# CompVis/stable-diffusion

Hardware: AMD Instinct MI355X
Metric: 512x512 images/sec, SD-v1-4 50-step PLMS CFG=7.5 (higher is better)
Workload: dtype f16

## Files before the change

### include/sdmi.h

```cpp
#ifndef SDMI_H_
#define SDMI_H_

#include <stdint.h>

#ifdef __cplusplus
extern "C" {
#endif

#define SDMI_ABI_VERSION 17

typedef struct sdmi_unet sdmi_unet;

typedef struct sdmi_unet_cfg {
  int32_t in_channels;
  int32_t out_channels;
  int32_t model_channels;
  int32_t num_res_blocks;
  int32_t n_levels;
  int32_t channel_mult[8];
  int32_t n_attention_resolutions;
  int32_t attention_resolutions[8];
  int32_t num_heads;
  int32_t transformer_depth;
  int32_t context_dim;
} sdmi_unet_cfg;

const char* sdmi_last_error(void);
int sdmi_abi_version(void);
int sdmi_has_experiments(void);

int sdmi_unet_create(const sdmi_unet_cfg* cfg, sdmi_unet** out);
#define SDMI_PRECISION_MIXED 0
#define SDMI_PRECISION_FULL 1
int sdmi_unet_create_with_precision(const sdmi_unet_cfg* cfg, int precision, sdmi_unet** out);
int sdmi_unet_precision(const sdmi_unet* h);
typedef struct sdmi_unet_ext {
  int32_t attention_block;
  int32_t resblock_updown;
} sdmi_unet_ext;
int sdmi_unet_create_ext(const sdmi_unet_cfg* cfg, const sdmi_unet_ext* ext, int precision, sdmi_unet** out);
#define SDMI_UNET_SCALE_SHIFT_NORM 1u
#define SDMI_UNET_NUM_HEAD_CHANNELS_SHIFT 16
#define SDMI_UNET_NUM_HEAD_CHANNELS_MASK 0x0fff0000u
#define SDMI_UNET_NUM_HEAD_CHANNELS(n) (((unsigned)(n) << SDMI_UNET_NUM_HEAD_CHANNELS_SHIFT) & SDMI_UNET_NUM_HEAD_CHANNELS_MASK)
int sdmi_unet_create_flags(const sdmi_unet_cfg* cfg, const sdmi_unet_ext* ext, unsigned flags, int precision, sdmi_unet** out);
int sdmi_unet_destroy(sdmi_unet* h);
int sdmi_unet_num_weights(const sdmi_unet* h);
int sdmi_unet_weight_info(const sdmi_unet* h, int idx, char* key_buf, int key_buf_len, int64_t* shape4, int* ndim);
int sdmi_unet_set_weight(sdmi_unet* h, const char* key, const float* ptr, const int64_t* shape, int ndim, void* stream);
int sdmi_unet_finalize(sdmi_unet* h);

int64_t sdmi_unet_packed_bytes(sdmi_unet* h);
int sdmi_unet_export_packed(sdmi_unet* h, void* host_buf, int64_t bytes, void* stream);
int sdmi_unet_import_packed(sdmi_unet* h, const void* host_buf, int64_t bytes, void* stream);

int64_t sdmi_unet_workspace_bytes(sdmi_unet* h, int B, int H, int W, int Lctx);

int sdmi_unet_cache_context(sdmi_unet* h, const float* ctx, int B, int Lctx, void* workspace, int64_t workspace_bytes,
                            void* stream);
int sdmi_unet_reserve_context(sdmi_unet* h, int B, int Lctx);

int sdmi_unet_cache_timesteps(sdmi_unet* h, const int64_t* t_host, int n, void* stream);
int sdmi_unet_hint_timestep(sdmi_unet* h, int64_t t);
int sdmi_unet_tape_stats(sdmi_unet* h, int64_t* replayed, int64_t* recorded);

int sdmi_unet_forward(sdmi_unet* h, const float* x, const int64_t* t_i64, const float* t_f32, const float* ctx,
                      float* eps_out, int B, int H, int W, int Lctx, void* workspace, int64_t workspace_bytes,
                      void* stream);

int sdmi_sampler_step(const float* eps_model, int cfg, float scale, const float* x, int mode, const float* old0,
                      const float* old1, const float* old2, float a_t, float a_prev, float sigma, float sqrt_1m_at,
                      const float* noise, float* e_t_out, float* x_prev, float* pred_x0, int64_t n, void* stream);


int sdmi_dpm_solver_step(const float* eps_model, int cfg, float scale, const float* x, const float* m_prev, float alpha_s,
                         float sigma_s, float cx, float a, float inv_r0, int order, float* m_out, float* x_next, int64_t n,
                         void* stream);

typedef struct sdmi_vae sdmi_vae;
typedef struct sdmi_vae_cfg {
  int32_t ch;
  int32_t out_ch;
  int32_t n_levels;
  int32_t ch_mult[8];
  int32_t num_res_blocks;
  int32_t in_channels;
  int32_t z_channels;
  int32_t embed_dim;
} sdmi_vae_cfg;
int sdmi_vae_create(const sdmi_vae_cfg* cfg, int parts, sdmi_vae** out);
typedef struct sdmi_vae_ext {
  int32_t double_z;
  int32_t mid_attn;
  int32_t n_embed;
} sdmi_vae_ext;
int sdmi_vae_create_ext(const sdmi_vae_cfg* cfg, const sdmi_vae_ext* ext, int parts, sdmi_vae** out);
int sdmi_vae_create_precision(const sdmi_vae_cfg* cfg, const sdmi_vae_ext* ext, int parts, int precision, sdmi_vae** out);
int sdmi_vae_precision(const sdmi_vae* h);
int sdmi_vae_decode_vq(sdmi_vae* h, const float* z, float z_scale, int quantize, float* img, int B, int H, int W, void* workspace,
                       int64_t workspace_bytes, void* stream);
int sdmi_vae_destroy(sdmi_vae* h);
int sdmi_vae_num_weights(const sdmi_vae* h);
int sdmi_vae_weight_info(const sdmi_vae* h, int idx, char* key_buf, int key_buf_len, int64_t* shape4, int* ndim);
int sdmi_vae_set_weight(sdmi_vae* h, const char* key, const float* ptr, const int64_t* shape, int ndim, void* stream);
int sdmi_vae_finalize(sdmi_vae* h);
int64_t sdmi_vae_decode_workspace_bytes(sdmi_vae* h, int B, int H, int W);
int sdmi_vae_decode(sdmi_vae* h, const float* z, float z_scale, float* img, int B, int H, int W, void* workspace,
                    int64_t workspace_bytes, void* stream);
int64_t sdmi_vae_encode_workspace_bytes(sdmi_vae* h, int B, int H, int W);
int sdmi_vae_encode(sdmi_vae* h, const float* img, float* moments, int B, int H, int W, void* workspace,
                    int64_t workspace_bytes, void* stream);


typedef struct sdmi_clip sdmi_clip;
typedef struct sdmi_clip_cfg {
  int32_t vocab_size;
  int32_t hidden_size;
  int32_t intermediate_size;
  int32_t num_layers;
  int32_t num_heads;
  int32_t max_positions;
} sdmi_clip_cfg;
int sdmi_clip_create(const sdmi_clip_cfg* cfg, sdmi_clip** out);
int sdmi_clip_destroy(sdmi_clip* h);
int sdmi_clip_num_weights(const sdmi_clip* h);
int sdmi_clip_weight_info(const sdmi_clip* h, int idx, char* key_buf, int key_buf_len, int64_t* shape4, int* ndim);
int sdmi_clip_set_weight(sdmi_clip* h, const char* key, const float* ptr, const int64_t* shape, int ndim, void* stream);
int sdmi_clip_finalize(sdmi_clip* h);
int64_t sdmi_clip_workspace_bytes(sdmi_clip* h, int B, int L);
int sdmi_clip_forward(sdmi_clip* h, const int64_t* ids, float* out, int B, int L, void* workspace, int64_t workspace_bytes,
                      void* stream);

typedef struct sdmi_bert sdmi_bert;
typedef struct sdmi_bert_cfg {
  int32_t vocab_size;
  int32_t dim;
  int32_t depth;
  int32_t heads;
  int32_t dim_head;
  int32_t ff_inner;
  int32_t max_seq_len;
} sdmi_bert_cfg;
int sdmi_bert_create(const sdmi_bert_cfg* cfg, sdmi_bert** out);
int sdmi_bert_destroy(sdmi_bert* h);
int sdmi_bert_num_weights(const sdmi_bert* h);
int sdmi_bert_weight_info(const sdmi_bert* h, int idx, char* key_buf, int key_buf_len, int64_t* shape4, int* ndim);
int sdmi_bert_set_weight(sdmi_bert* h, const char* key, const float* ptr, const int64_t* shape, int ndim, void* stream);
int sdmi_bert_finalize(sdmi_bert* h);
int64_t sdmi_bert_workspace_bytes(sdmi_bert* h, int B, int L);
int sdmi_bert_forward(sdmi_bert* h, const int64_t* ids, float* out, int B, int L, void* workspace, int64_t workspace_bytes,
                      void* stream);

typedef struct sdmi_igemm_desc {
  const void* a0; const void* a1; const void* a2;
  int32_t c0, c1, c2, lda0, lda1, lda2;
  int32_t B, Hin, Win, Hout, Wout, ksize, stride, up;
  const void* w;
  int32_t N;
  int32_t mode;
  const float* bias; const float* rowvec; int32_t ld_rowvec;
  const float* residual; int32_t ldr;
  float* out_f32; void* out_f16; int32_t ldo;
  void* seg_dst[3]; int32_t seg_kind[3];
  int32_t heads, dh, ntok, ntok_pad, segC;
  int32_t splitk;
  float* splitk_ws; int64_t splitk_ws_floats;
  int32_t tile;
  int32_t dma;
  int32_t asym_pad;
  int32_t gn_n; void* gn_acc[2]; int32_t gn_cpg[2]; int32_t gn_cbase[2];
  int32_t* splitk_cnt; int32_t splitk_cnt_ints;
  int32_t split16;
  const float* f16_scale; float* lnp_out;
  const float* lnf_part; int32_t lnf_npart; float lnf_eps; const float* lnf_cs; const float* lnf_d;
  const float* pgn_gamma; const float* pgn_beta; float pgn_eps; int32_t pgn_silu;
  void* pgn_out; int32_t pgn_keep_f32; int32_t* pgn_applied;
  void* out_lo;
} sdmi_igemm_desc;
int sdmi_k_igemm(const sdmi_igemm_desc* d, void* stream);
int sdmi_k_ff_tail(const sdmi_igemm_desc* proj_out, const void* ln_f16, const float* lnp, float ln_eps, const float* csd,
                   const void* wgg_f16, const void* wff2_f16, const float* bff2, const float* t, void* stream);
int sdmi_k_st_tail(const sdmi_igemm_desc* proj_out, const void* a_f16, const void* wo_f16, const float* bo, float* t, const float* ln_gamma,
                   float ln_eps, const float* csd, const void* wgg_f16, const void* wff2_f16, const float* bff2, void* stream);
int sdmi_k_gn_conv3(const sdmi_igemm_desc* conv, const float* x0, const float* x1, int c0, int c1, float* gn_ws, int64_t gn_ws_floats,
                    const float* gn_gamma, const float* gn_beta, float gn_eps, void* stream);
int sdmi_k_st_head(const float* x, float* gn_ws, int64_t gn_ws_floats, const float* gn_gamma, const float* gn_beta, float gn_eps,
                   const void* w_in3, const float* b_in, float* t, const float* ln_gamma, float ln_eps, const void* wqkv_f16,
                   const float* lnf_cs, const float* lnf_d, void* q, void* k, void* vt, int B, int ntok, int ntok_pad, int heads, int dh,
                   int C, void* stream);
int sdmi_k_st_mid(const void* a_f16, const void* wo_f16, const float* bo, float* t, const float* ln_gamma, float ln_eps, const void* wq_f16,
                  const float* lnf_cs, const float* lnf_d, void* q, int B, int ntok, int heads, int dh, int C, void* stream);
int sdmi_k_st_mid_ctx(const void* a_f16, const void* wo_f16, const float* bo, float* t, const float* ln_gamma, float ln_eps, const void* wq_f16,
                      const float* lnf_cs, const float* lnf_d, const void* ctx_k, const void* ctx_vt, int nkv, int nkv_pad, float scale, void* ao_out,
                      int B, int ntok, int heads, int dh, int C, void* stream);
int sdmi_k_ln_fold_prep(const void* w_f16, int N, int K, int ldw, const float* gamma, const float* beta, const float* bias,
                        float* cs, float* d, void* stream);
int sdmi_k_attention(const void* q, const void* k, const void* vt, void* out, int BH, int heads, int nq, int nkv,
                     int nkv_pad, int d, float scale, void* stream);
int sdmi_k_attention_split16(const void* q, const void* q_lo, const void* k, const void* k_lo, const void* vt, const void* vt_lo, void* out,
                             void* out_lo, int BH, int heads, int nq, int nkv, int nkv_pad, int d, float scale, void* stream);
int sdmi_k_attention_causal(const void* q, const void* k, const void* vt, void* out, int BH, int heads, int n, int n_pad,
                            int d, float scale, void* stream);
int sdmi_k_groupnorm(const float* x0, const float* x1, int c0, int c1, int B, int HW, const float* gamma,
                     const float* beta, float eps, int silu, void* out_f16, float* out_f32, void* raw_f16, void* out_lo,
                     void* raw_lo, float* partial_ws, int64_t partial_floats, void* stream);
int64_t sdmi_k_groupnorm_ws_floats(int B, int HW);
int sdmi_k_groupnorm_film(const float* x0, const float* x1, int c0, int c1, int B, int HW, const float* gamma, const float* beta, float eps,
                          int silu, const float* film, int film_ld, void* out_f16, float* out_f32, void* raw_f16, void* out_lo, void* raw_lo,
                          float* partial_ws, int64_t partial_floats, void* stream);
int sdmi_k_layernorm(const float* x, const float* gamma, const float* beta, void* out_f16, int M, int C, float eps,
                     void* stream);
int sdmi_k_cast_f16(const float* x, void* out_f16, void* out_lo, int64_t n, void* stream);
int sdmi_k_split_heads(const float* src, int ld, int col0, void* dst, void* dst_lo, int kind, int B, int ntok, int ntok_pad, int heads, int dh,
                       void* stream);
int sdmi_k_geglu_split(const float* src, int M, int F, void* out, void* out_lo, void* stream);
int sdmi_k_layernorm_split(const float* x, const float* gamma, const float* beta, void* out, void* out_lo, int M, int C, float eps, void* stream);
int sdmi_k_timestep_embedding(const int64_t* t_i64, const float* t_f32, float* out, int B, int dim, void* stream);
int sdmi_k_small_linear(const float* in, int ld_in, const float* w, const float* bias, float* out, int ld_out, int B,
                        int N, int K, int silu_in, void* stream);
int sdmi_k_conv_in(const float* x_nchw, const float* w_oihw, const float* bias, float* out_nhwc, int B, int Cin, int H,
                   int W, int Cout, void* stream);
int sdmi_k_conv_out(const float* h_nhwc, const float* w_ohwi, const float* bias, float* out_nchw, int B, int H, int W,
                    int Cin, int Cout, void* stream);
int sdmi_k_pack_conv_weight(const float* w_oihw, void* dst_f16, int O, int I, int KH, int KW, void* stream);
int sdmi_k_pack_conv_weight_src(const float* w_oihw, void* dst_f16, int O, int I, int KH, int KW, int c0, int c1, int c2, void* stream);
int sdmi_k_pack_conv_out(const float* w_oihw, float* dst_ohwi, int O, int I, void* stream);
int sdmi_k_pack_split3(const float* w, void* dst_f16, int N, int K, void* stream);
int sdmi_k_pack_conv_split3(const float* w_oihw, void* dst_f16, int O, int I, int KH, int KW, void* stream);
int sdmi_k_pointwise_nchw(const float* x, const float* w, const float* bias, float* out, int B, int Cin, int Cout, int HW,
                          float in_scale, void* stream);
int sdmi_k_softmax_rows(const float* S, void* P_f16, int rows, int cols, float scale, void* stream);
int sdmi_k_vq_quantize(const float* z, float z_scale, const float* codebook, float* norms_ws, int n_embed, int D, float* zq, int32_t* idx,
                       int B, int HW, void* stream);
int sdmi_k_resample2(const float* x, float* out_f32, void* out_f16, void* out_lo, int B, int H, int W, int C, int dir, void* stream);
int sdmi_k_patch_unfold(const float* x, const float* c, float* out, int B, int Cx, int Cc, int H, int W, int kh, int kw, int sy, int sx,
                        int l0, int nl, void* stream);
int sdmi_k_patch_fold(const float* o, const float* w, float* out, int B, int C, int H, int W, int kh, int kw, int sy, int sx, int uf, int df,
                      int norm_only, void* stream);
int sdmi_k_gelu_erf(const float* x, void* out_f16, int64_t n, void* stream);
int sdmi_k_pack_geglu(const float* w, const float* bias, void* wdst_f16, float* bdst, int N, int K, void* stream);
int sdmi_image_to_uint8(const float* img_nchw, void* out_nhwc_u8, int B, int C, int H, int W, void* stream);
int sdmi_range_check(int enable);
int sdmi_range_report(char* json_buf, int json_buf_len);
int sdmi_tune_begin(void);
int sdmi_tune_round(int r);
int sdmi_tune_end(const char* path, int* n_keys);
int sdmi_tune_dump(char* buf, int buflen);
int sdmi_profile_begin(void);
int sdmi_profile_end(char* json_buf, int json_buf_len);
int sdmi_k_prefetch_lines(const void* ptr, int64_t bytes, void* stream);
const void* sdmi_zero_page(void);

#ifdef __cplusplus
}
#endif
#endif
```

### stable-diffusion_amd/_lib.py

```python
import ctypes as C
import os

_HERE = os.path.dirname(os.path.abspath(__file__))
LIB_PATH = os.environ.get('SDMI_LIB_PATH') or os.path.join(_HERE, 'libsdmi.so')

c_f32p = C.c_void_p
c_ptr = C.c_void_p


class UNetCfg(C.Structure):
    _fields_ = [('in_channels', C.c_int32), ('out_channels', C.c_int32), ('model_channels', C.c_int32),
                ('num_res_blocks', C.c_int32), ('n_levels', C.c_int32), ('channel_mult', C.c_int32 * 8),
                ('n_attention_resolutions', C.c_int32), ('attention_resolutions', C.c_int32 * 8),
                ('num_heads', C.c_int32), ('transformer_depth', C.c_int32), ('context_dim', C.c_int32)]


class VaeCfg(C.Structure):
    _fields_ = [('ch', C.c_int32), ('out_ch', C.c_int32), ('n_levels', C.c_int32), ('ch_mult', C.c_int32 * 8),
                ('num_res_blocks', C.c_int32), ('in_channels', C.c_int32), ('z_channels', C.c_int32),
                ('embed_dim', C.c_int32)]


class UNetExt(C.Structure):
    _fields_ = [('attention_block', C.c_int32), ('resblock_updown', C.c_int32)]
# ... 20 lines not shown
                ('B', C.c_int32), ('Hin', C.c_int32), ('Win', C.c_int32), ('Hout', C.c_int32), ('Wout', C.c_int32),
                ('ksize', C.c_int32), ('stride', C.c_int32), ('up', C.c_int32),
                ('w', c_ptr), ('N', C.c_int32), ('mode', C.c_int32),
                ('bias', c_ptr), ('rowvec', c_ptr), ('ld_rowvec', C.c_int32),
                ('residual', c_ptr), ('ldr', C.c_int32),
                ('out_f32', c_ptr), ('out_f16', c_ptr), ('ldo', C.c_int32),
                ('seg_dst', c_ptr * 3), ('seg_kind', C.c_int32 * 3),
                ('heads', C.c_int32), ('dh', C.c_int32), ('ntok', C.c_int32), ('ntok_pad', C.c_int32),
                ('segC', C.c_int32), ('splitk', C.c_int32), ('splitk_ws', c_ptr), ('splitk_ws_floats', C.c_int64),
                ('tile', C.c_int32), ('dma', C.c_int32), ('asym_pad', C.c_int32),
                ('gn_n', C.c_int32), ('gn_acc', c_ptr * 2), ('gn_cpg', C.c_int32 * 2), ('gn_cbase', C.c_int32 * 2),
                ('splitk_cnt', c_ptr), ('splitk_cnt_ints', C.c_int32), ('split16', C.c_int32),
                ('f16_scale', c_ptr), ('lnp_out', c_ptr), ('lnf_part', c_ptr), ('lnf_npart', C.c_int32),
                ('lnf_eps', C.c_float), ('lnf_cs', c_ptr), ('lnf_d', c_ptr),
                ('pgn_gamma', c_ptr), ('pgn_beta', c_ptr), ('pgn_eps', C.c_float), ('pgn_silu', C.c_int32),
                ('pgn_out', c_ptr), ('pgn_keep_f32', C.c_int32), ('pgn_applied', C.POINTER(C.c_int32)),
                ('out_lo', c_ptr)]


_SIGS = {
    'sdmi_last_error': (C.c_char_p, []),
    'sdmi_abi_version': (C.c_int, []),
    'sdmi_unet_create': (C.c_int, [C.POINTER(UNetCfg), C.POINTER(c_ptr)]),
    'sdmi_unet_create_with_precision': (C.c_int, [C.POINTER(UNetCfg), C.c_int, C.POINTER(c_ptr)]),
    'sdmi_unet_precision': (C.c_int, [c_ptr]),
    'sdmi_unet_create_ext': (C.c_int, [C.POINTER(UNetCfg), C.POINTER(UNetExt), C.c_int, C.POINTER(c_ptr)]),
    'sdmi_unet_create_flags': (C.c_int, [C.POINTER(UNetCfg), C.POINTER(UNetExt), C.c_uint, C.c_int, C.POINTER(c_ptr)]),
    'sdmi_unet_destroy': (C.c_int, [c_ptr]),
    'sdmi_unet_num_weights': (C.c_int, [c_ptr]),
    'sdmi_unet_weight_info': (C.c_int, [c_ptr, C.c_int, C.c_char_p, C.c_int, C.POINTER(C.c_int64), C.POINTER(C.c_int)]),
    'sdmi_unet_set_weight': (C.c_int, [c_ptr, C.c_char_p, c_ptr, C.POINTER(C.c_int64), C.c_int, c_ptr]),
    'sdmi_unet_finalize': (C.c_int, [c_ptr]),
    'sdmi_unet_packed_bytes': (C.c_int64, [c_ptr]),
    'sdmi_unet_export_packed': (C.c_int, [c_ptr, c_ptr, C.c_int64, c_ptr]),
    'sdmi_unet_import_packed': (C.c_int, [c_ptr, c_ptr, C.c_int64, c_ptr]),
    'sdmi_unet_workspace_bytes': (C.c_int64, [c_ptr, C.c_int, C.c_int, C.c_int, C.c_int]),
    'sdmi_unet_cache_context': (C.c_int, [c_ptr, c_ptr, C.c_int, C.c_int, c_ptr, C.c_int64, c_ptr]),
    'sdmi_unet_reserve_context': (C.c_int, [c_ptr, C.c_int, C.c_int]),
    'sdmi_unet_cache_timesteps': (C.c_int, [c_ptr, C.POINTER(C.c_int64), C.c_int, c_ptr]),
    'sdmi_unet_hint_timestep': (C.c_int, [c_ptr, C.c_int64]),
    'sdmi_unet_tape_stats': (C.c_int, [c_ptr, C.POINTER(C.c_int64), C.POINTER(C.c_int64)]),
    'sdmi_unet_forward': (C.c_int, [c_ptr, c_ptr, c_ptr, c_ptr, c_ptr, c_ptr, C.c_int, C.c_int, C.c_int, C.c_int,
                                    c_ptr, C.c_int64, c_ptr]),
    'sdmi_sampler_step': (C.c_int, [c_ptr, C.c_int, C.c_float, c_ptr, C.c_int, c_ptr, c_ptr, c_ptr, C.c_float,
                                    C.c_float, C.c_float, C.c_float, c_ptr, c_ptr, c_ptr, c_ptr, C.c_int64, c_ptr]),
    'sdmi_dpm_solver_step': (C.c_int, [c_ptr, C.c_int, C.c_float, c_ptr, c_ptr, C.c_float, C.c_float, C.c_float, C.c_float,
                                       C.c_float, C.c_int, c_ptr, c_ptr, C.c_int64, c_ptr]),
    'sdmi_vae_create': (C.c_int, [C.POINTER(VaeCfg), C.c_int, C.POINTER(c_ptr)]),
    'sdmi_vae_destroy': (C.c_int, [c_ptr]),
    'sdmi_vae_create_ext': (C.c_int, [C.POINTER(VaeCfg), C.POINTER(VaeExt), C.c_int, C.POINTER(c_ptr)]),
    'sdmi_vae_create_precision': (C.c_int, [C.POINTER(VaeCfg), C.POINTER(VaeExt), C.c_int, C.c_int, C.POINTER(c_ptr)]),
    'sdmi_vae_precision': (C.c_int, [c_ptr]),
    'sdmi_vae_decode_vq': (C.c_int, [c_ptr, c_ptr, C.c_float, C.c_int, c_ptr, C.c_int, C.c_int, C.c_int, c_ptr, C.c_int64, c_ptr]),
    'sdmi_k_vq_quantize': (C.c_int, [c_ptr, C.c_float, c_ptr, c_ptr, C.c_int, C.c_int, c_ptr, c_ptr, C.c_int, C.c_int, c_ptr]),
    'sdmi_k_patch_unfold': (C.c_int, [c_ptr, c_ptr, c_ptr] + [C.c_int] * 11 + [c_ptr]),
    'sdmi_k_patch_fold': (C.c_int, [c_ptr, c_ptr, c_ptr] + [C.c_int] * 11 + [c_ptr]),
    'sdmi_k_resample2': (C.c_int, [c_ptr, c_ptr, c_ptr, c_ptr, C.c_int, C.c_int, C.c_int, C.c_int, C.c_int, c_ptr]),
    'sdmi_vae_num_weights': (C.c_int, [c_ptr]),
    'sdmi_vae_weight_info': (C.c_int, [c_ptr, C.c_int, C.c_char_p, C.c_int, C.POINTER(C.c_int64), C.POINTER(C.c_int)]),
    'sdmi_vae_set_weight': (C.c_int, [c_ptr, C.c_char_p, c_ptr, C.POINTER(C.c_int64), C.c_int, c_ptr]),
    'sdmi_vae_finalize': (C.c_int, [c_ptr]),
    'sdmi_vae_decode_workspace_bytes': (C.c_int64, [c_ptr, C.c_int, C.c_int, C.c_int]),
    'sdmi_vae_decode': (C.c_int, [c_ptr, c_ptr, C.c_float, c_ptr, C.c_int, C.c_int, C.c_int, c_ptr, C.c_int64, c_ptr]),
    'sdmi_vae_encode_workspace_bytes': (C.c_int64, [c_ptr, C.c_int, C.c_int, C.c_int]),
    'sdmi_vae_encode': (C.c_int, [c_ptr, c_ptr, c_ptr, C.c_int, C.c_int, C.c_int, c_ptr, C.c_int64, c_ptr]),
    'sdmi_clip_create': (C.c_int, [C.POINTER(ClipCfg), C.POINTER(c_ptr)]),
    'sdmi_clip_destroy': (C.c_int, [c_ptr]),
    'sdmi_clip_num_weights': (C.c_int, [c_ptr]),
    'sdmi_clip_weight_info': (C.c_int, [c_ptr, C.c_int, C.c_char_p, C.c_int, C.POINTER(C.c_int64), C.POINTER(C.c_int)]),
    'sdmi_clip_set_weight': (C.c_int, [c_ptr, C.c_char_p, c_ptr, C.POINTER(C.c_int64), C.c_int, c_ptr]),
    'sdmi_clip_finalize': (C.c_int, [c_ptr]),
    'sdmi_clip_workspace_bytes': (C.c_int64, [c_ptr, C.c_int, C.c_int]),
    'sdmi_clip_forward': (C.c_int, [c_ptr, c_ptr, c_ptr, C.c_int, C.c_int, c_ptr, C.c_int64, c_ptr]),
    'sdmi_bert_create': (C.c_int, [C.POINTER(BertCfg), C.POINTER(c_ptr)]),
    'sdmi_bert_destroy': (C.c_int, [c_ptr]),
    'sdmi_bert_num_weights': (C.c_int, [c_ptr]),
    'sdmi_bert_weight_info': (C.c_int, [c_ptr, C.c_int, C.c_char_p, C.c_int, C.POINTER(C.c_int64), C.POINTER(C.c_int)]),
    'sdmi_bert_set_weight': (C.c_int, [c_ptr, C.c_char_p, c_ptr, C.POINTER(C.c_int64), C.c_int, c_ptr]),
    'sdmi_bert_finalize': (C.c_int, [c_ptr]),
    'sdmi_bert_workspace_bytes': (C.c_int64, [c_ptr, C.c_int, C.c_int]),
    'sdmi_bert_forward': (C.c_int, [c_ptr, c_ptr, c_ptr, C.c_int, C.c_int, c_ptr, C.c_int64, c_ptr]),
    'sdmi_has_experiments': (C.c_int, []),
    'sdmi_k_igemm': (C.c_int, [C.POINTER(IGemmDesc), c_ptr]),
    'sdmi_k_ff_tail': (C.c_int, [C.POINTER(IGemmDesc), c_ptr, c_ptr, C.c_float, c_ptr, c_ptr, c_ptr, c_ptr, c_ptr, c_ptr]),
    'sdmi_k_gn_conv3': (C.c_int, [C.POINTER(IGemmDesc), c_ptr, c_ptr, C.c_int, C.c_int, c_ptr, C.c_int64, c_ptr, c_ptr, C.c_float, c_ptr]),
    'sdmi_k_st_mid_ctx': (C.c_int, [c_ptr, c_ptr, c_ptr, c_ptr, c_ptr, C.c_float, c_ptr, c_ptr, c_ptr, c_ptr, c_ptr, C.c_int, C.c_int, C.c_float, c_ptr,
                                    C.c_int, C.c_int, C.c_int, C.c_int, C.c_int, c_ptr]),
    'sdmi_k_st_tail': (C.c_int, [C.POINTER(IGemmDesc), c_ptr, c_ptr, c_ptr, c_ptr, c_ptr, C.c_float, c_ptr, c_ptr, c_ptr, c_ptr, c_ptr]),
    'sdmi_k_st_mid': (C.c_int, [c_ptr, c_ptr, c_ptr, c_ptr, c_ptr, C.c_float, c_ptr, c_ptr, c_ptr, c_ptr, C.c_int, C.c_int, C.c_int, C.c_int,
                                C.c_int, c_ptr]),
    'sdmi_k_st_head': (C.c_int, [c_ptr, c_ptr, C.c_int64, c_ptr, c_ptr, C.c_float, c_ptr, c_ptr, c_ptr, c_ptr, C.c_float, c_ptr, c_ptr, c_ptr,
                                 c_ptr, c_ptr, c_ptr, C.c_int, C.c_int, C.c_int, C.c_int, C.c_int, C.c_int, c_ptr]),
    'sdmi_k_attention_split16': (C.c_int, [c_ptr, c_ptr, c_ptr, c_ptr, c_ptr, c_ptr, c_ptr, c_ptr, C.c_int, C.c_int, C.c_int, C.c_int,
                                           C.c_int, C.c_int, C.c_float, c_ptr]),
    'sdmi_k_attention_causal': (C.c_int, [c_ptr, c_ptr, c_ptr, c_ptr, C.c_int, C.c_int, C.c_int, C.c_int, C.c_int, C.c_float,
                                          c_ptr]),
    'sdmi_k_pointwise_nchw': (C.c_int, [c_ptr, c_ptr, c_ptr, c_ptr, C.c_int, C.c_int, C.c_int, C.c_int, C.c_float, c_ptr]),
    'sdmi_k_softmax_rows': (C.c_int, [c_ptr, c_ptr, C.c_int, C.c_int, C.c_float, c_ptr]),
    'sdmi_k_gelu_erf': (C.c_int, [c_ptr, c_ptr, C.c_int64, c_ptr]),
    'sdmi_k_attention': (C.c_int, [c_ptr, c_ptr, c_ptr, c_ptr, C.c_int, C.c_int, C.c_int, C.c_int, C.c_int, C.c_int,
                                   C.c_float, c_ptr]),
    'sdmi_k_groupnorm': (C.c_int, [c_ptr, c_ptr, C.c_int, C.c_int, C.c_int, C.c_int, c_ptr, c_ptr, C.c_float, C.c_int,
                                   c_ptr, c_ptr, c_ptr, c_ptr, c_ptr, c_ptr, C.c_int64, c_ptr]),
    'sdmi_k_groupnorm_ws_floats': (C.c_int64, [C.c_int, C.c_int]),
    'sdmi_k_groupnorm_film': (C.c_int, [c_ptr, c_ptr, C.c_int, C.c_int, C.c_int, C.c_int, c_ptr, c_ptr, C.c_float, C.c_int, c_ptr, C.c_int,
                                        c_ptr, c_ptr, c_ptr, c_ptr, c_ptr, c_ptr, C.c_int64, c_ptr]),
    'sdmi_k_layernorm': (C.c_int, [c_ptr, c_ptr, c_ptr, c_ptr, C.c_int, C.c_int, C.c_float, c_ptr]),
    'sdmi_k_cast_f16': (C.c_int, [c_ptr, c_ptr, c_ptr, C.c_int64, c_ptr]),
    'sdmi_k_split_heads': (C.c_int, [c_ptr, C.c_int, C.c_int, c_ptr, c_ptr, C.c_int, C.c_int, C.c_int, C.c_int, C.c_int, C.c_int,
                                     c_ptr]),
    'sdmi_k_geglu_split': (C.c_int, [c_ptr, C.c_int, C.c_int, c_ptr, c_ptr, c_ptr]),
    'sdmi_k_layernorm_split': (C.c_int, [c_ptr, c_ptr, c_ptr, c_ptr, c_ptr, C.c_int, C.c_int, C.c_float, c_ptr]),
    'sdmi_k_timestep_embedding': (C.c_int, [c_ptr, c_ptr, c_ptr, C.c_int, C.c_int, c_ptr]),
    'sdmi_k_small_linear': (C.c_int, [c_ptr, C.c_int, c_ptr, c_ptr, c_ptr, C.c_int, C.c_int, C.c_int, C.c_int,
                                      C.c_int, c_ptr]),
    'sdmi_k_conv_in': (C.c_int, [c_ptr, c_ptr, c_ptr, c_ptr, C.c_int, C.c_int, C.c_int, C.c_int, C.c_int, c_ptr]),
    'sdmi_k_conv_out': (C.c_int, [c_ptr, c_ptr, c_ptr, c_ptr, C.c_int, C.c_int, C.c_int, C.c_int, C.c_int, c_ptr]),
    'sdmi_k_pack_conv_weight': (C.c_int, [c_ptr, c_ptr, C.c_int, C.c_int, C.c_int, C.c_int, c_ptr]),
    'sdmi_k_pack_conv_weight_src': (C.c_int, [c_ptr, c_ptr, C.c_int, C.c_int, C.c_int, C.c_int, C.c_int, C.c_int, C.c_int, c_ptr]),
    'sdmi_k_pack_conv_out': (C.c_int, [c_ptr, c_ptr, C.c_int, C.c_int, c_ptr]),
    'sdmi_k_pack_split3': (C.c_int, [c_ptr, c_ptr, C.c_int, C.c_int, c_ptr]),
    'sdmi_k_pack_conv_split3': (C.c_int, [c_ptr, c_ptr, C.c_int, C.c_int, C.c_int, C.c_int, c_ptr]),
    'sdmi_k_pack_geglu': (C.c_int, [c_ptr, c_ptr, c_ptr, c_ptr, C.c_int, C.c_int, c_ptr]),
    'sdmi_k_ln_fold_prep': (C.c_int, [c_ptr, C.c_int, C.c_int, C.c_int, c_ptr, c_ptr, c_ptr, c_ptr, c_ptr, c_ptr]),
    'sdmi_image_to_uint8': (C.c_int, [c_ptr, c_ptr, C.c_int, C.c_int, C.c_int, C.c_int, c_ptr]),
    'sdmi_range_check': (C.c_int, [C.c_int]),
    'sdmi_range_report': (C.c_int, [C.c_char_p, C.c_int]),
    'sdmi_tune_begin': (C.c_int, []),
    'sdmi_tune_round': (C.c_int, [C.c_int]),
    'sdmi_tune_end': (C.c_int, [C.c_char_p, C.POINTER(C.c_int)]),
    'sdmi_tune_dump': (C.c_int, [C.c_char_p, C.c_int]),
    'sdmi_profile_begin': (C.c_int, []),
    'sdmi_profile_end': (C.c_int, [C.c_char_p, C.c_int]),
    'sdmi_k_prefetch_lines': (C.c_int, [c_ptr, C.c_int64, c_ptr]),
    'sdmi_zero_page': (c_ptr, []),
}

_lib = None


class SdmiError(RuntimeError):
    pass


def load():
    global _lib
    if _lib is None:
        if not os.path.exists(LIB_PATH):
            raise SdmiError(f'{LIB_PATH} not found: build it with `python stable-diffusion_amd/build.py` '
                            '(the MI355X path has no fallback implementation)')
        lib = C.CDLL(LIB_PATH)
        for name, (res, args) in _SIGS.items():
            fn = getattr(lib, name)
            fn.restype = res
            fn.argtypes = args
        if lib.sdmi_abi_version() != 17:
            raise SdmiError('libsdmi ABI version mismatch')
        _lib = lib
    return _lib


def exported_symbols():
    return sorted(_SIGS)


def check(rc):
# ... 12 lines not shown
```

### stable-diffusion_amd/csrc/api.cpp

```cpp
#include <string.h>

#include <new>

#include "prof.h"
#include "split16.h"
#include "unet.h"
#include "vae.h"
#include "clip.h"

namespace sdmi {
static thread_local std::string g_err;
void set_error(const std::string& msg) { g_err = msg; }
int fail(const std::string& msg) { g_err = msg; return -1; }
}

struct sdmi_unet { sdmi::UNet impl; };
struct sdmi_vae { sdmi::Vae impl; };
struct sdmi_clip { sdmi::ClipText impl; };
struct sdmi_bert { sdmi::BertText impl; };

using namespace sdmi;

static int weight_info(const WeightStore& w, int idx, char* key_buf, int key_buf_len, int64_t* shape4, int* ndim) {
  SDMI_CHECK(key_buf && shape4 && ndim, "null argument");
// ... 247 lines not shown
  *out = h;
  return 0;
}
int sdmi_bert_destroy(sdmi_bert* h) { delete h; return 0; }
int sdmi_bert_num_weights(const sdmi_bert* h) { return h ? (int)h->impl.weights().slots().size() : fail("null handle"); }
int sdmi_bert_weight_info(const sdmi_bert* h, int idx, char* key_buf, int key_buf_len, int64_t* shape4, int* ndim) {
  SDMI_CHECK(h, "null argument");
  return weight_info(h->impl.weights(), idx, key_buf, key_buf_len, shape4, ndim);
}
int sdmi_bert_set_weight(sdmi_bert* h, const char* key, const float* ptr, const int64_t* shape, int ndim, void* stream) {
  SDMI_CHECK(h && key && ptr && shape, "null argument");
  return h->impl.set_weight(key, ptr, shape, ndim, (hipStream_t)stream);
}
int sdmi_bert_finalize(sdmi_bert* h) { SDMI_CHECK(h, "null handle"); return h->impl.finalize(); }
int64_t sdmi_bert_workspace_bytes(sdmi_bert* h, int B, int L) {
  if (!h) { fail("null handle"); return 0; }
  int64_t need = 0;
  if (h->impl.forward(nullptr, nullptr, B, L, nullptr, 0, nullptr, true, &need)) return 0;
  return need;
}
int sdmi_bert_forward(sdmi_bert* h, const int64_t* ids, float* out, int B, int L, void* workspace, int64_t workspace_bytes,
                      void* stream) {
  SDMI_CHECK(h && ids && out, "null argument");
  return h->impl.forward(ids, out, B, L, workspace, workspace_bytes, (hipStream_t)stream, false, nullptr);
}
int sdmi_k_vq_quantize(const float* z, float z_scale, const float* codebook, float* norms_ws, int n_embed, int D, float* zq, int32_t* idx,
                       int B, int HW, void* stream) {
  if (launch_vq_norms(codebook, norms_ws, n_embed, D, (hipStream_t)stream)) return -1;
  return launch_vq_quantize(z, z_scale, codebook, norms_ws, n_embed, D, zq, (int*)idx, B, HW, (hipStream_t)stream);
}
int sdmi_k_resample2(const float* x, float* out_f32, void* out_f16, void* out_lo, int B, int H, int W, int C, int dir, void* stream) {
  return launch_resample2(x, out_f32, (f16*)out_f16, (f16*)out_lo, B, H, W, C, dir, (hipStream_t)stream);
}
int sdmi_k_patch_unfold(const float* x, const float* c, float* out, int B, int Cx, int Cc, int H, int W, int kh, int kw, int sy, int sx,
                        int l0, int nl, void* stream) {
  return launch_patch_unfold(x, c, out, B, Cx, Cc, H, W, kh, kw, sy, sx, l0, nl, (hipStream_t)stream);
}
int sdmi_k_patch_fold(const float* o, const float* w, float* out, int B, int C, int H, int W, int kh, int kw, int sy, int sx, int uf, int df,
                      int norm_only, void* stream) {
  return launch_patch_fold(o, w, out, B, C, H, W, kh, kw, sy, sx, uf, df, norm_only, (hipStream_t)stream);
}
int sdmi_k_gelu_erf(const float* x, void* out_f16, int64_t n, void* stream) {
  return launch_gelu_erf(x, (f16*)out_f16, n, (hipStream_t)stream);
}
int sdmi_k_attention_causal(const void* q, const void* k, const void* vt, void* out, int BH, int heads, int n, int n_pad,
                            int d, float scale, void* stream) {
  AttnParams a = AttnParams();
  a.q = (const f16*)q; a.k = (const f16*)k; a.vt = (const f16*)vt; a.out = (f16*)out;
  a.BH = BH; a.heads = heads; a.nq = n; a.nkv = n; a.nkv_pad = n_pad; a.d = d; a.scale = scale; a.causal = 1;
  return launch_attention(a, (hipStream_t)stream);
}

static int igemm_params_of(const sdmi_igemm_desc* d, IGemmParams& p) {
  p.a0 = (const f16*)d->a0; p.a1 = (const f16*)d->a1; p.a2 = (const f16*)d->a2;
  p.c0 = d->c0; p.c1 = d->c1; p.c2 = d->c2; p.lda0 = d->lda0; p.lda1 = d->lda1; p.lda2 = d->lda2;
  p.B = d->B; p.Hin = d->Hin; p.Win = d->Win; p.Hout = d->Hout; p.Wout = d->Wout;
  p.ksize = d->ksize; p.stride = d->stride; p.up = d->up; p.pad = d->asym_pad ? 0 : 1;
  p.w = (const f16*)d->w; p.M = d->B * d->Hout * d->Wout; p.N = d->N; p.K = d->ksize * d->ksize * (d->c0 + d->c1 + d->c2);
  p.mode = d->mode; p.bias = d->bias; p.rowvec = d->rowvec; p.ld_rowvec = d->ld_rowvec;
  p.residual = d->residual; p.ldr = d->ldr; p.out_f32 = d->out_f32; p.out_f16 = (f16*)d->out_f16; p.ldo = d->ldo;
  for (int i = 0; i < 3; ++i) { p.seg_dst[i] = (f16*)d->seg_dst[i]; p.seg_kind[i] = d->seg_kind[i]; }
  p.heads = d->heads; p.dh = d->dh; p.ntok = d->ntok; p.ntok_pad = d->ntok_pad; p.segC = d->segC;
  p.splitk = d->splitk; p.splitk_ws = d->splitk_ws; p.splitk_ws_floats = d->splitk_ws_floats;
  p.splitk_cnt = d->splitk_cnt; p.splitk_cnt_ints = d->splitk_cnt_ints;
  p.gn_n = d->gn_n;
  for (int i = 0; i < 2; ++i) { p.gn_acc[i] = (long long*)d->gn_acc[i]; p.gn_cpg[i] = d->gn_cpg[i]; p.gn_cbase[i] = d->gn_cbase[i]; }
  if (d->split16) {
    p.split16 = 1; p.c1 = 0; p.K = d->c0; p.ldw = 3 * d->c0;
  }
  p.f16_scale = d->f16_scale; p.lnp_out = d->lnp_out;
  p.lnf_part = d->lnf_part; p.lnf_npart = d->lnf_npart; p.lnf_eps = d->lnf_eps; p.lnf_cs = d->lnf_cs; p.lnf_d = d->lnf_d;
  p.pgn_gamma = d->pgn_gamma; p.pgn_beta = d->pgn_beta; p.pgn_eps = d->pgn_eps; p.pgn_silu = d->pgn_silu;
  p.pgn_out = (f16*)d->pgn_out; p.pgn_keep_f32 = d->pgn_keep_f32; p.pgn_applied = d->pgn_applied;
  p.out_lo = (f16*)d->out_lo;
  return zero_page(&p.zero_page);
}
int sdmi_k_igemm(const sdmi_igemm_desc* d, void* stream) {
  SDMI_CHECK(d, "null descriptor");
  IGemmParams p = IGemmParams();
  if (igemm_params_of(d, p)) return -1;
  IGemmTune t; t.tile = d->tile; t.dma = d->dma;
  return launch_igemm(p, t, (hipStream_t)stream);
}
int sdmi_k_ff_tail(const sdmi_igemm_desc* proj_out, const void* ln_f16, const float* lnp, float ln_eps, const float* csd,
                   const void* wgg_f16, const void* wff2_f16, const float* bff2, const float* t, void* stream) {
  SDMI_CHECK(proj_out, "null descriptor");
  FfTailParams q = FfTailParams();
  if (igemm_params_of(proj_out, q.epi)) return -1;
  SDMI_CHECK(proj_out->split16 && proj_out->ksize == 1, "ff_tail: the proj_out descriptor is a split-fp16 1x1 (w = sdmi_k_pack_split3)");
  q.ln = (const f16*)ln_f16; q.lnp = lnp; q.ln_eps = ln_eps; q.csd = csd; q.wgg = (const f16*)wgg_f16; q.wff2 = (const f16*)wff2_f16;
  q.bff2 = bff2; q.t = t; q.wpo = (const f16*)proj_out->w;
  return launch_ff_tail(q, (hipStream_t)stream);
}
int sdmi_k_st_tail(const sdmi_igemm_desc* proj_out, const void* a_f16, const void* wo_f16, const float* bo, float* t, const float* ln_gamma,
                   float ln_eps, const float* csd, const void* wgg_f16, const void* wff2_f16, const float* bff2, void* stream) {
  SDMI_CHECK(proj_out && a_f16, "null argument");
  FfTailParams q = FfTailParams();
  if (igemm_params_of(proj_out, q.epi)) return -1;
  SDMI_CHECK(proj_out->split16 && proj_out->ksize == 1, "st_tail: the proj_out descriptor is a split-fp16 1x1 (w = sdmi_k_pack_split3)");
  q.a16 = (const f16*)a_f16; q.wo = (const f16*)wo_f16; q.bo = bo; q.ln_gamma = ln_gamma; q.ln_eps = ln_eps; q.csd = csd;
  q.wgg = (const f16*)wgg_f16; q.wff2 = (const f16*)wff2_f16; q.bff2 = bff2; q.t = t; q.wpo = (const f16*)proj_out->w;
  return launch_ff_tail(q, (hipStream_t)stream);
}
int sdmi_k_gn_conv3(const sdmi_igemm_desc* conv, const float* x0, const float* x1, int c0, int c1, float* gn_ws, int64_t gn_ws_floats,
                    const float* gn_gamma, const float* gn_beta, float gn_eps, void* stream) {
  SDMI_CHECK(conv && x0 && gn_ws && gn_gamma && gn_beta, "gn_conv3: null argument");
  GnConvParams q = GnConvParams();
  if (igemm_params_of(conv, q.epi)) return -1;
  const int B = q.epi.B;
  SDMI_CHECK(gn_ws_floats >= gn_acc_words(B) * 2, "groupnorm workspace too small");
  SDMI_HIP_OK(hipMemsetAsync(gn_ws, 0, gn_acc_words(B) * sizeof(long long), (hipStream_t)stream));
  GroupNormParams g = GroupNormParams();
  g.x0 = x0; g.c0 = c0; g.x1 = x1; g.c1 = c1; g.B = B; g.HW = q.epi.Hout * q.epi.Wout; g.gamma = gn_gamma; g.beta = gn_beta; g.eps = gn_eps;
  g.stats_only = 1; g.acc = (long long*)gn_ws;
  if (launch_groupnorm(g, (hipStream_t)stream)) return -1;
  q.x0 = x0; q.x1 = x1; q.c0 = c0; q.c1 = c1; q.gn_acc = (const long long*)gn_ws; q.gn_gamma = gn_gamma; q.gn_beta = gn_beta; q.gn_eps = gn_eps;
  q.w = (const f16*)conv->w;
  return launch_gn_conv3(q, (hipStream_t)stream);
}
int sdmi_k_st_head(const float* x, float* gn_ws, int64_t gn_ws_floats, const float* gn_gamma, const float* gn_beta, float gn_eps,
                   const void* w_in3, const float* b_in, float* t, const float* ln_gamma, float ln_eps, const void* wqkv_f16,
                   const float* lnf_cs, const float* lnf_d, void* q, void* k, void* vt, int B, int ntok, int ntok_pad, int heads, int dh,
                   int C, void* stream) {
  SDMI_CHECK(x && gn_ws && gn_gamma && gn_beta, "st_head: null argument");
  SDMI_CHECK(gn_ws_floats >= gn_acc_words(B) * 2, "groupnorm workspace too small");
  SDMI_HIP_OK(hipMemsetAsync(gn_ws, 0, gn_acc_words(B) * sizeof(long long), (hipStream_t)stream));
  GroupNormParams g = GroupNormParams();
  g.x0 = x; g.c0 = C; g.B = B; g.HW = ntok; g.gamma = gn_gamma; g.beta = gn_beta; g.eps = gn_eps; g.stats_only = 1; g.acc = (long long*)gn_ws;
  if (launch_groupnorm(g, (hipStream_t)stream)) return -1;
  StHeadParams p = StHeadParams();
  p.x = x; p.gn_acc = (const long long*)gn_ws; p.gn_gamma = gn_gamma; p.gn_beta = gn_beta; p.gn_eps = gn_eps;
  p.w_in = (const f16*)w_in3; p.b_in = b_in; p.t = t; p.ln_gamma = ln_gamma; p.ln_eps = ln_eps; p.wqkv = (const f16*)wqkv_f16;
  p.lnf_cs = lnf_cs; p.lnf_d = lnf_d; p.q = (f16*)q; p.k = (f16*)k; p.vt = (f16*)vt;
  p.M = B * ntok; p.B = B; p.ntok = ntok; p.ntok_pad = ntok_pad; p.heads = heads; p.dh = dh; p.C = C;
  return launch_st_head(p, (hipStream_t)stream);
}
int sdmi_k_st_mid(const void* a_f16, const void* wo_f16, const float* bo, float* t, const float* ln_gamma, float ln_eps, const void* wq_f16,
                  const float* lnf_cs, const float* lnf_d, void* q, int B, int ntok, int heads, int dh, int C, void* stream) {
  StHeadParams p = StHeadParams();
  p.a16 = (const f16*)a_f16; p.w_in = (const f16*)wo_f16; p.b_in = bo; p.t = t; p.ln_gamma = ln_gamma; p.ln_eps = ln_eps;
  p.wqkv = (const f16*)wq_f16; p.lnf_cs = lnf_cs; p.lnf_d = lnf_d; p.q = (f16*)q;
  p.M = B * ntok; p.B = B; p.ntok = ntok; p.ntok_pad = ntok; p.heads = heads; p.dh = dh; p.C = C;
  return launch_st_mid(p, (hipStream_t)stream);
}
int sdmi_k_st_mid_ctx(const void* a_f16, const void* wo_f16, const float* bo, float* t, const float* ln_gamma, float ln_eps, const void* wq_f16,
                      const float* lnf_cs, const float* lnf_d, const void* ctx_k, const void* ctx_vt, int nkv, int nkv_pad, float scale, void* ao_out,
                      int B, int ntok, int heads, int dh, int C, void* stream) {
  StHeadParams p = StHeadParams();
  p.a16 = (const f16*)a_f16; p.w_in = (const f16*)wo_f16; p.b_in = bo; p.t = t; p.ln_gamma = ln_gamma; p.ln_eps = ln_eps;
  p.wqkv = (const f16*)wq_f16; p.lnf_cs = lnf_cs; p.lnf_d = lnf_d;
  p.ctx_k = (const f16*)ctx_k; p.ctx_vt = (const f16*)ctx_vt; p.ctx_nkv = nkv; p.ctx_nkv_pad = nkv_pad; p.ctx_scale = scale; p.ao_out = (f16*)ao_out;
  SDMI_CHECK(ctx_k && ctx_vt && ao_out, "st_mid_ctx: null argument");
  p.M = B * ntok; p.B = B; p.ntok = ntok; p.ntok_pad = ntok; p.heads = heads; p.dh = dh; p.C = C;
  return launch_st_mid(p, (hipStream_t)stream);
}
int sdmi_k_ln_fold_prep(const void* w_f16, int N, int K, int ldw, const float* gamma, const float* beta, const float* bias,
                        float* cs, float* d, void* stream) {
  return launch_ln_fold_prep((const f16*)w_f16, N, K, ldw, gamma, beta, bias, cs, d, (hipStream_t)stream);
}
int sdmi_k_attention(const void* q, const void* k, const void* vt, void* out, int BH, int heads, int nq, int nkv,
                     int nkv_pad, int d, float scale, void* stream) {
  AttnParams a = AttnParams();
  a.q = (const f16*)q; a.k = (const f16*)k; a.vt = (const f16*)vt; a.out = (f16*)out;
  a.BH = BH; a.heads = heads; a.nq = nq; a.nkv = nkv; a.nkv_pad = nkv_pad; a.d = d; a.scale = scale;
  if (const char* e = getenv("SDMI_ATTN_NW")) a.nw = atoi(e);
  return launch_attention(a, (hipStream_t)stream);
// ... 127 lines not shown
```

### stable-diffusion_amd/csrc/common.h

```cpp
#pragma once
#include <hip/hip_runtime.h>
#include <stdint.h>
#include <algorithm>
#include <string>

#include "tape.h"

typedef _Float16 f16;
typedef _Float16 f16x2 __attribute__((ext_vector_type(2)));
typedef _Float16 f16x4 __attribute__((ext_vector_type(4)));
typedef _Float16 f16x8 __attribute__((ext_vector_type(8)));
typedef float f32x4 __attribute__((ext_vector_type(4)));
typedef float f32x16 __attribute__((ext_vector_type(16)));

#ifdef __HIPCC__
__device__ __forceinline__ float gn_apply_elem(float v, float mean, float rstd, float gamma, float beta, int silu) {
  float t = __builtin_fmaf((v - mean) * rstd, gamma, beta);
  if (silu) t = t * __builtin_amdgcn_rcpf(1.0f + __expf(-t));
  return t;
}
__device__ __forceinline__ float gn_apply_film_elem(float v, float mean, float rstd, float gamma, float beta, float scale, float shift,
                                                    int silu) {
  float t = __builtin_fmaf((v - mean) * rstd, gamma, beta);
  t = __builtin_fmaf(t, 1.0f + scale, shift);
// ... 67 lines not shown
    __builtin_amdgcn_raw_buffer_store_b128(__builtin_bit_cast(sdmi_u32x4, v), r, (int)byte_off, 0, 16);
  } else {
    *(f32x4*)((char*)base + byte_off) = v;
  }
}
__device__ __forceinline__ void sdmi_st_wt8(const void* base, size_t byte_off, f16x4 v) {
  if (__builtin_expect(byte_off < (size_t)0x80000000u - 16, 1)) {
    const __amdgpu_buffer_rsrc_t r = __builtin_amdgcn_make_buffer_rsrc((void*)base, 0, (int)0x80000000, 0x00020000);
    __builtin_amdgcn_raw_buffer_store_b64(__builtin_bit_cast(sdmi_u32x2, v), r, (int)byte_off, 0, 16);
  } else {
    *(f16x4*)((char*)base + byte_off) = v;
  }
}
#define SDMI_ST_F32X4(base, off, val) sdmi_st_wt16((base), (size_t)(off) * 4, (val))
#if SDMI_WT_STORES >= 2
#define SDMI_ST_F16X4(base, off, val) sdmi_st_wt8((base), (size_t)(off) * 2, (val))
#else
#define SDMI_ST_F16X4(base, off, val) SDMI_ST(f16x4, (base) + (off), (val))
#endif
#else
#define SDMI_ST_F32X4(base, off, val) SDMI_ST(f32x4, (base) + (off), (val))
#define SDMI_ST_F16X4(base, off, val) SDMI_ST(f16x4, (base) + (off), (val))
#endif

struct IGemmParams {
  const f16* a0 = nullptr; const f16* a1 = nullptr; const f16* a2 = nullptr;
  int c0 = 0, c1 = 0, c2 = 0;
  int lda0 = 0, lda1 = 0, lda2 = 0;
  int B = 1, Hin = 1, Win = 1;
  int Hout = 1, Wout = 1;
  int ksize = 1, stride = 1, up = 0;
  int pad = 1;
  const f16* w = nullptr;
  int M = 0, N = 0, K = 0;
  int k_alg = 0;
  int split16 = 0;
  int ldw = 0;
  int mode = EPI_PLAIN;
  const float* bias = nullptr;
  const float* rowvec = nullptr; int ld_rowvec = 0;
  const float* residual = nullptr; int ldr = 0;
  float* out_f32 = nullptr; f16* out_f16 = nullptr; int ldo = 0;
  f16* out_lo = nullptr;
  const float* ln_gamma = nullptr; const float* ln_beta = nullptr; f16* ln_out = nullptr; float ln_eps = 1e-5f;
  const float* f16_scale = nullptr;
  float* lnp_out = nullptr;
  const float* lnf_part = nullptr; int lnf_npart = 0; float lnf_eps = 1e-5f;
  const float* lnf_cs = nullptr; const float* lnf_d = nullptr;
  f16* seg_dst[3] = {nullptr, nullptr, nullptr};
  int seg_kind[3] = {0, 0, 0};
  int heads = 0, dh = 0, ntok = 0, ntok_pad = 0, segC = 0;
  int splitk = 1;
  float* splitk_ws = nullptr; int64_t splitk_ws_floats = 0;
  int* splitk_cnt = nullptr; int splitk_cnt_ints = 0;
  int nkt = 0;
#ifdef SDMI_IGEMM_TIMING
  long long* dbg_times = nullptr;
  int dbg_abl = 0;
#endif
  int splitk_fused = 0;
  int slab_tiled = 0, slab_bm = 0, slab_bn = 0, slab_wm = 0, slab_wn = 0;
  int slab_sh_qpt = 0, slab_sh_nt = 0, slab_sh_tn = 0, slab_sh_wn = 0;
  int epi_vec = 0;
  int tile_n_fastest = 0;
  const f16* zero_page = nullptr;
  int gn_n = 0;
  long long* gn_acc[2] = {nullptr, nullptr};
  int gn_cpg[2] = {0, 0}, gn_cbase[2] = {0, 0};
  unsigned long long gn_magic[2] = {0, 0};
  const float* pgn_gamma = nullptr; const float* pgn_beta = nullptr; float pgn_eps = 1e-5f; int pgn_silu = 1;
  f16* pgn_out = nullptr;
  int pgn_keep_f32 = 0;
  int* pgn_applied = nullptr;
  unsigned long long magic_hw = 0, magic_w = 0, magic_w2 = 0;
  int log2w = 0;
  const float* xf0 = nullptr; const float* xf1 = nullptr;
  const long long* gn_in_acc = nullptr;
  const float* gn_in_gamma = nullptr; const float* gn_in_beta = nullptr; float gn_in_eps = 1e-5f; int gn_in_silu = 1;
  f16* raw_hi = nullptr; f16* raw_lo = nullptr;
  f16* gn_scratch = nullptr;
  unsigned long long magic_cpg_in = 0;
  int halo_thi = 0, halo_ipt = 1, log2_tpi = 30;
  unsigned long long magic_hpi = 0;
};

constexpr int SDMI_NUM_TILES = 22;
struct IGemmTune {
  int tile = -1;
  int dma = -1;
};

int launch_igemm(const IGemmParams& p, const IGemmTune& tune, hipStream_t stream);
bool range_check_enabled();
uint64_t tune_generation();
bool tune_collecting();
int range_check_set(int enable);
int range_scan(const char* what, const f16* p, int64_t n, hipStream_t stream);
int range_report(std::string* json);

int tune_begin();
int tune_round(int r);
int tune_end(const char* path, int* n_keys);
int tune_dump(std::string* out);
int launch_splitk_reduce(const IGemmParams& p, int nsplit, hipStream_t stream);

struct FfTailParams {
  const f16* ln = nullptr;
  const float* lnp = nullptr;
  float ln_eps = 1e-5f;
  const float* csd = nullptr;
  const f16* wgg = nullptr;
  const f16* wff2 = nullptr;
  const float* bff2 = nullptr;
  const float* t = nullptr;
  const f16* wpo = nullptr;
  const f16* a16 = nullptr;
  const f16* wo = nullptr;
  const float* bo = nullptr;
  const float* ln_gamma = nullptr;
#ifdef SDMI_RC_TIMING
  long long* dbg = nullptr;
#endif
  IGemmParams epi;
};
bool ff_tail_supported(int C, int M, int rows_per_sample);
int launch_ff_tail(const FfTailParams& p, hipStream_t stream);

struct StHeadParams {
  const f16* a16 = nullptr;
  const float* x = nullptr;
  const long long* gn_acc = nullptr;
  const float* gn_gamma = nullptr; const float* gn_beta = nullptr; float gn_eps = 1e-6f;
  const f16* w_in = nullptr;
  const float* b_in = nullptr;
  float* t = nullptr;
  const float* ln_gamma = nullptr;
  float ln_eps = 1e-5f;
  const f16* wqkv = nullptr;
  const float* lnf_cs = nullptr; const float* lnf_d = nullptr;
  f16* q = nullptr; f16* k = nullptr;
  f16* vt = nullptr;
  int M = 0, B = 0, ntok = 0, ntok_pad = 0, heads = 0, dh = 0, C = 0;
  const f16* ctx_k = nullptr; const f16* ctx_vt = nullptr; int ctx_nkv = 0, ctx_nkv_pad = 0; float ctx_scale = 0.f; f16* ao_out = nullptr;
#ifdef SDMI_RC_TIMING
  long long* dbg = nullptr;
#endif
};
bool st_head_supported(int C, int M, int ntok, int ntok_pad, int heads, int dh);
int launch_st_head(const StHeadParams& p, hipStream_t stream);
int launch_st_mid(const StHeadParams& p, hipStream_t stream);

struct GnConvParams {
  const float* x0 = nullptr; const float* x1 = nullptr; int c0 = 0, c1 = 0;
  const long long* gn_acc = nullptr;
  const float* gn_gamma = nullptr; const float* gn_beta = nullptr; float gn_eps = 1e-5f;
  const f16* w = nullptr;
#ifdef SDMI_RC_TIMING
  long long* dbg = nullptr;
#endif
  IGemmParams epi;
};
bool gn_conv3_supported(int B, int H, int W, int c0, int c1, int Cout);
int launch_gn_conv3(const GnConvParams& p, hipStream_t stream);

struct AttnParams {
  const f16* q = nullptr;
  const f16* k = nullptr;
  const f16* vt = nullptr;
  f16* out = nullptr;
  int BH = 0, heads = 0, nq = 0, nkv = 0, nkv_pad = 0, d = 0;
  float scale = 1.f;
  int nw = 0;
  int causal = 0;
  int prio = 0;
  int pingpong = 0;
// ... 102 lines not shown
```

### stable-diffusion_amd/csrc/conv3halo.hip

```cpp
#include "igemm_dev.h"

namespace sdmi {
namespace {

template <int BM, int BN, int WARPS_M, int WARPS_N, int NS>
__global__ void __launch_bounds__(WARPS_M* WARPS_N * 64) conv3halo_kernel(const IGemmParams p, const int tiles_m,
                                                                           const int tiles_n, const int chunks_per_split) {
#if defined(__HIP_DEVICE_COMPILE__)
  constexpr int NT = WARPS_M * WARPS_N * 64;
  constexpr int RPP = NT / 8;
  constexpr int PB = BN / RPP;
  constexpr int WTM = BM / WARPS_M, WTN = BN / WARPS_N;
  constexpr int TM = WTM / 32, TN = WTN / 32;
  constexpr int HPMAX = (BM / 64 + 2) * 66;
  constexpr int AHP = (HPMAX + RPP - 1) / RPP;
  constexpr int HALO_BYTES = AHP * RPP * 128;
  constexpr int BSTAGE = BN * 128;
  constexpr int LDS_BYTES = 2 * HALO_BYTES + NS * BSTAGE;
  constexpr int LASTA = 10 - NS;
  constexpr int PA = (AHP + LASTA) / (LASTA + 1);
  constexpr int KS = BK / 16;
  constexpr int G = (TM * TN >= 4) ? 1 : 2;
  constexpr int U = KS / G;
  constexpr int MPU = G * TM * TN;
  static_assert(PB >= 1 && TM >= 1 && TN >= 1 && RPP % 16 == 0 && NS >= 2 && NS <= 9, "tile/wave shape");
  static_assert(LDS_BYTES <= 160 * 1024, "LDS budget");

  __shared__ __attribute__((aligned(16))) unsigned char smem[LDS_BYTES];

  const int nblk = gridDim.x;
  const int bid = blockIdx.x;
  const int q8 = nblk >> 3, r8 = nblk & 7, xcd = bid & 7;
  const int wgid = (xcd < r8 ? xcd * (q8 + 1) : r8 * (q8 + 1) + (xcd - r8) * q8) + (bid >> 3);
  const int tiles_mn = tiles_m * tiles_n;
  const int split = wgid / tiles_mn;
  const int tmn = wgid - split * tiles_mn;
  int tile_m, tile_n;
  if (p.tile_n_fastest) { tile_m = tmn / tiles_n; tile_n = tmn - tile_m * tiles_n; }
  else { tile_n = tmn / tiles_m; tile_m = tmn - tile_n * tiles_m; }
  const int m0 = tile_m * BM, n0 = tile_n * BN;
  const int nch = (p.c0 + p.c1 + p.c2) / BK;
  const int c_begin = split * chunks_per_split;
  const int c_end = min(nch, c_begin + chunks_per_split);
  if (c_begin >= c_end) return;

  const int tid = threadIdx.x;
  SDMI_STAMP(dbg_t0);
  const int lane = tid & 63;
  const int wave = tid >> 6;
  const int cpos = tid & 7, lrow = tid >> 3;
  const int gch = cpos ^ ((lrow >> 1) & 7);
  const int wave_u = __builtin_amdgcn_readfirstlane(wave);
  const int wm = wave / WARPS_N, wn = wave - wm * WARPS_N;
  const int l31 = lane & 31, lg = lane >> 5;
  const int rsw = (l31 >> 1) & 7;

  const int W = p.Wout, H = p.Hout, HW = H * W, W2 = W + 2, ld = p.lda0;
  const int bimg = m0 / HW;
  const int THI = p.halo_thi;
  const int HPI = (THI + 2) * W2;
  const int y0 = p.halo_ipt > 1 ? 0 : (m0 - bimg * HW) >> p.log2w;
  const int HP = p.halo_ipt * HPI;
  constexpr int OOB = (int)0x80000000;

  int hvoff[AHP];
#pragma unroll
  for (int q = 0; q < AHP; ++q) {
    const int hp = q * RPP + lrow;
    const int ip = fast_div(hp, p.magic_hpi), hr = hp - ip * HPI;
    const int hy = fast_div(hr, p.magic_w2), hx = hr - hy * W2;
    const int y = y0 + hy - 1, x = hx - 1;
    const bool valid = hp < HP && y >= 0 && y < H && x >= 0 && x < W;
    hvoff[q] = valid ? ((((bimg + ip) * H + y) * W + x) * ld + gch * 8) * 2 : OOB;
  }
  int b_off[PB];
#pragma unroll
  for (int i = 0; i < PB; ++i) {
    const int n = min(n0 + i * RPP + lrow, p.N - 1);
    b_off[i] = (n * p.K + gch * 8) * 2;
  }
  int hr0[TM];
#pragma unroll
  for (int i = 0; i < TM; ++i) {
    const int ml = wm * WTM + i * 32 + l31;
    const int ip = ml >> p.log2_tpi, mr = ml & ((1 << p.log2_tpi) - 1);
    hr0[i] = ip * HPI + (mr >> p.log2w) * W2 + (mr & (W - 1));
  }
  const int b_lds = 2 * HALO_BYTES + (wn * WTN + l31) * 128;
// ... 49 lines not shown

  auto a_lo = [](int t) { return t <= LASTA ? (t * PA < AHP ? t * PA : AHP) : AHP; };
  auto a_hi = [](int t) { return t <= LASTA ? ((t + 1) * PA < AHP ? (t + 1) * PA : AHP) : AHP; };
  auto in_flight_ok = [&](int t) {
    int n = 0;
    for (int d = 0; d < NS - 2; ++d) { const int tt = (t - d + 18) % 9; n += a_hi(tt) - a_lo(tt) + PB; }
    return n;
  };

  const int kt_first = c_begin * 9, kt_last = c_end * 9 - 1;
  {
    const ChunkSrc cs = chunk_src(c_begin);
#pragma unroll
    for (int q = 0; q < AHP; ++q) issue_halo(cs, 0, q);
#pragma unroll
    for (int s2 = 0; s2 < NS - 1; ++s2) {
      const int vt = 9 - (NS - 1) + s2;
#pragma unroll
      for (int e = a_lo(vt); e < a_hi(vt); ++e) issue_halo(cs, 0, 0);
#pragma unroll
      for (int q = 0; q < PB; ++q) issue_b(min(kt_first + s2, kt_last), s2, q);
    }
  }
  wait_vmcnt_n(in_flight_ok(8));
  asm volatile("s_waitcnt lgkmcnt(0)\n\ts_barrier" ::: "memory");
  SDMI_STAMP(dbg_t1);
  f16x8 fa[2][G][TM], fb[2][G][TN];
  int ab[TM];
#pragma unroll
  for (int i = 0; i < TM; ++i) ab[i] = a_base(i, 0, 0, 0);
#pragma unroll
  for (int g = 0; g < G; ++g) read_frags(ab, 0, g, fa[0][g], fb[0][g]);

  int cur = 0, nxt = NS - 1, hb = 0;
  for (int c = c_begin; c < c_end; ++c) {
    const ChunkSrc csn = chunk_src(min(c + 1, c_end - 1));
#pragma unroll
    for (int tap = 0; tap < 9; ++tap) {
      const int kt = c * 9 + tap;
      const int tap1 = tap == 8 ? 0 : tap + 1;
      const int hb1 = tap == 8 ? (hb ^ 1) : hb;
      const int cur1 = (cur + 1 == NS) ? 0 : cur + 1;
      int ab1[TM];
#pragma unroll
      for (int i = 0; i < TM; ++i) ab1[i] = a_base(i, tap1 / 3, tap1 % 3, hb1);
      const int alo = a_lo(tap);
      const int na = a_hi(tap) - alo;
      const int npieces = na + PB;
      const int ppu = (npieces + U - 2) / (U - 1);
      const int bt = min(kt + NS - 1, kt_last);
#pragma unroll
      for (int u = 0; u < U; ++u) {
        if (u + 1 < U) {
#pragma unroll
          for (int g = 0; g < G; ++g) read_frags(ab, cur, (u + 1) * G + g, fa[(u + 1) & 1][g], fb[(u + 1) & 1][g]);
#pragma unroll
          for (int e = u * ppu; e < (u + 1) * ppu && e < npieces; ++e) {
            if (e < na) issue_halo(csn, hb ^ 1, alo + e);
            else issue_b(bt, nxt, e - na);
          }
        } else {
          wait_vmcnt_n(in_flight_ok(tap));
          asm volatile("s_waitcnt lgkmcnt(0)\n\ts_barrier" ::: "memory");
#pragma unroll
          for (int g = 0; g < G; ++g) read_frags(ab1, cur1, g, fa[0][g], fb[0][g]);
        }
#pragma unroll
        for (int g = 0; g < G; ++g) mfma_step(fa[u & 1][g], fb[u & 1][g]);
        __builtin_amdgcn_sched_group_barrier(0x100, G * (TM + TN), 0);
#pragma unroll
        for (int e = 0; e < MPU; ++e) {
          __builtin_amdgcn_sched_group_barrier(0x008, 1, 0);
          if (u + 1 < U && e < ppu && u * ppu + e < npieces) __builtin_amdgcn_sched_group_barrier(0x010, 1, 0);
        }
      }
#pragma unroll
      for (int i = 0; i < TM; ++i) ab[i] = ab1[i];
      cur = cur1;
      nxt = (nxt + 1 == NS) ? 0 : nxt + 1;
      hb = hb1;
    }
  }
  wait_vmcnt<0>();
  SDMI_STAMP(dbg_t2);
  igemm_epilogue<BM, BN, WARPS_M, WARPS_N, LDS_BYTES>(p, acc, m0, n0, split, tile_m, tile_n, smem);
#ifdef SDMI_IGEMM_TIMING
  if (p.dbg_times && tid == 0) {
    long long* d = p.dbg_times + 6 * (size_t)blockIdx.x;
    d[0] = dbg_t0; d[1] = dbg_t1; d[2] = dbg_t2; d[4] = (long long)__builtin_readcyclecounter();
  }
#endif
#endif
}

}

bool halo_supported(const IGemmParams& p, int bm) {
  const int W = p.Wout, HW = p.Hout * p.Wout;
  if (p.c0 % BK || p.c1 % BK || p.c2 % BK) return false;
  if (!(p.ksize == 3 && p.stride == 1 && p.pad == 1 && !p.up && p.Hin == p.Hout && p.Win == p.Wout && W >= 8 && W <= 64 &&
        (W & (W - 1)) == 0 && bm % W == 0))
    return false;
  const int cap = (((bm / 64 + 2) * 66 + bm / 4 - 1) / (bm / 4)) * (bm / 4);
  if (bm <= HW) return HW % bm == 0 && (bm / W + 2) * (W + 2) <= cap;
  return bm % HW == 0 && p.M % bm == 0 && (bm / HW) * (p.Hout + 2) * (W + 2) <= cap;
}

template <int BM, int BN, int WARPS_M, int WARPS_N, int NS>
int launch_halo_cfg(const IGemmParams& p, int splitk, hipStream_t stream) {
  SDMI_CHECK(halo_supported(p, BM), "halo-staged conv tile requested for an unsupported shape");
  const int tiles_m = cdiv(p.M, BM), tiles_n = cdiv(p.N, BN);
  const int nch = (p.c0 + p.c1 + p.c2) / BK;
  const int chunks_per_split = cdiv(nch, splitk);
  const int nsplit = cdiv(nch, chunks_per_split);
  IGemmParams q = p;
  q.splitk = nsplit;
  q.tile_n_fastest = tile_order_n_fastest(p);
  q.splitk_fused = 0;
  slab_layout(q, BM, BN, WARPS_M, WARPS_N, nsplit);
  q.epi_vec = epi_vec_ok(p);
  SDMI_CHECK(splitk_ws_need(p, BM, BN, nsplit) <= p.splitk_ws_floats, "split-K workspace too small");
  SDMI_CHECK((int64_t)p.M < (int64_t)65536 * p.Hout * p.Wout, "fast_div_hw: at most 65535 samples per launch");
  q.magic_hw = div_magic_hw(p.Hout * p.Wout);
  q.magic_w = div_magic(p.Wout);
  q.magic_w2 = div_magic(p.Wout + 2);
  q.log2w = 0;
  while ((1 << q.log2w) < p.Wout) ++q.log2w;
  {
    const int HW = p.Hout * p.Wout;
    q.halo_ipt = BM <= HW ? 1 : BM / HW;
    q.halo_thi = BM <= HW ? BM / p.Wout : p.Hout;
    q.magic_hpi = div_magic((q.halo_thi + 2) * (p.Wout + 2));
    const int tpi = q.halo_thi * p.Wout;
    q.log2_tpi = 0;
    while ((1 << q.log2_tpi) < tpi) ++q.log2_tpi;
    if (q.halo_ipt == 1) q.log2_tpi = 30;
  }
  for (int t = 0; t < p.gn_n; ++t) q.gn_magic[t] = div_magic(p.gn_cpg[t]);
  dim3 grid(tiles_m * tiles_n * nsplit), block(WARPS_M * WARPS_N * 64);
  static const int by_shape = env_int("SDMI_PROF_SHAPES", 0);
  std::string pname = std::string("conv3halo_") + std::to_string(BM) + "x" + std::to_string(BN) + "w" +
                      std::to_string(WARPS_M * WARPS_N) + "s" + std::to_string(NS);
  if (by_shape && prof_enabled())
    pname += "_M" + std::to_string(p.M) + "_N" + std::to_string(p.N) + "_K" + std::to_string(p.K) + "_s" + std::to_string(nsplit);
  const double src_pix = (double)p.B * p.Hin * p.Win;
  ProfScope ps(pname.c_str(), 2.0 * p.M * (double)p.N * p.K,
               src_pix * (p.c0 + p.c1) * 2.0 + (double)p.N * p.K * 2.0 + (double)p.M * p.N * ((p.out_f32 ? 4.0 : 0.0) + (p.out_f16 ? 2.0 : 0.0)) +
                   (p.residual ? (double)p.M * p.N * 4.0 : 0.0),
               stream);
  SDMI_LAUNCH((conv3halo_kernel<BM, BN, WARPS_M, WARPS_N, NS>), grid, block, 0, stream, q, tiles_m, tiles_n, chunks_per_split);
  SDMI_HIP_OK(hipGetLastError());
  ps.end();
  if (nsplit > 1) return launch_splitk_reduce(q, nsplit, stream);
  if (q.ln_out) return launch_layernorm(q.out_f32, q.ln_gamma, q.ln_beta, q.ln_out, q.M, q.N, q.ln_eps, stream);
  return 0;
}

int launch_halo_tile(int tile, const IGemmParams& p, int splitk, hipStream_t stream) {
  switch (tile) {
    case 14: return launch_halo_cfg<256, 64, 4, 2, 5>(p, splitk, stream);
    case 15: return launch_halo_cfg<256, 128, 4, 2, 3>(p, splitk, stream);
    case 16: return launch_halo_cfg<128, 64, 2, 2, 8>(p, splitk, stream);
    case 17: return launch_halo_cfg<128, 128, 2, 2, 5>(p, splitk, stream);
    default: return fail("not a halo-staged conv tile id");
  }
}

}
```

### stable-diffusion_amd/csrc/igemm.hip

```cpp
#include <dlfcn.h>

#include <map>
#include <mutex>
#include <tuple>
#include <vector>

#include "igemm_dev.h"

namespace sdmi {
namespace {

__global__ void __launch_bounds__(256) splitk_reduce_kernel(IGemmParams p, int nsplit, int rows_per_block) {
  __shared__ unsigned long long s_gn[2][32][GN_WORDS];
  const int tx = threadIdx.x & 7, ty = threadIdx.x >> 3;
  const int n = (blockIdx.x * 8 + tx) * 4;
  const int row0 = blockIdx.y * rows_per_block;
  const int HW = p.Hout * p.Wout;
  const bool gn = p.gn_n > 0;
  const bool ncol = n < p.N;
  if (gn) {
    for (int i = threadIdx.x; i < 2 * 32 * GN_WORDS; i += 256) (&s_gn[0][0][0])[i] = 0ull;
    __syncthreads();
  }
  const size_t slab_sz = (size_t)p.M * p.N;
// ... 295 lines not shown

int launch_splitk_reduce(const IGemmParams& p, int nsplit, hipStream_t stream) {
  SDMI_CHECK(nsplit >= 1 && nsplit <= 16 && p.N % 4 == 0 && p.splitk_ws, "splitk_reduce: bad arguments");
  if (p.slab_tiled) {
    const int64_t quads = (int64_t)cdiv(p.M, p.slab_bm) * cdiv(p.N, p.slab_bn) * (p.slab_bm * p.slab_bn / 4);
    SDMI_CHECK(quads % 256 == 0 && quads / 256 < (1ll << 31) && p.slab_wm > 0 && p.slab_wn > 0, "tiled split-K slabs: bad geometry");
    const double mn = (double)p.M * p.N;
    if (p.mode == EPI_HEADS) {
      ProfScope psh("splitk_reduce", 0.0, mn * (4.0 * nsplit + 2.0), stream);
      SDMI_LAUNCH(splitk_reduce_tiled_heads_kernel, dim3((unsigned)(quads / 256)), dim3(256), 0, stream, p, nsplit);
      SDMI_HIP_OK(hipGetLastError());
      return 0;
    }
    if (p.gn_n > 0) SDMI_CHECK((p.Hout * p.Wout) % 32 == 0, "GroupNorm statistics need Hout*Wout % 32 == 0");
    const bool coop = env_int("SDMI_REDUCE_GN_XCD", SDMI_REDUCE_GN_XCD_DEFAULT) && p.pgn_out && p.pgn_gamma && p.pgn_beta && p.mode == EPI_PLAIN && p.gn_n == 1 &&
                      p.gn_cbase[0] == 0 && p.gn_cpg[0] == p.N / 32 && p.N % 128 == 0 && p.N / 32 >= 16 && p.M == p.B * p.Hout * p.Wout &&
                      (p.Hout * p.Wout) % 32 == 0 && !p.out_f16 && !p.out_lo && !p.ln_out && p.splitk_cnt && p.splitk_cnt_ints >= COOP_BAR_INTS &&
                      quads % 1024 == 0 && quads / 1024 <= 256 && (!p.pgn_keep_f32 || (p.out_f32 && p.ldo % 4 == 0));
    ProfScope pst(coop ? "splitk_reduce_gn" : "splitk_reduce", 0.0, coop ? mn * (4.0 * nsplit + 2.0 + (p.pgn_keep_f32 ? 4.0 : 0.0)) : mn * 4.0 * (nsplit + 1), stream);
    const int rb_env = env_int("SDMI_REDUCE_BLOCK", 256);
    const int rb = (rb_env == 128 || (rb_env == 0 && quads / 256 < 512)) ? 128 : 256;
    if (coop) {
      SDMI_LAUNCH(splitk_reduce_tiled_kernel<true>, dim3((unsigned)(quads / 1024)), dim3(1024), 0, stream, p, nsplit);
      SDMI_HIP_OK(hipGetLastError());
      pst.end();
      if (p.pgn_applied) *p.pgn_applied = 1;
      if (range_check_enabled() && range_scan("GroupNorm fp16 output (split-K reduction)", p.pgn_out, (int64_t)p.M * p.N, stream)) return -1;
      return 0;
    }
    SDMI_LAUNCH(splitk_reduce_tiled_kernel<false>, dim3((unsigned)(quads / rb)), dim3(rb), 0, stream, p, nsplit);
    SDMI_HIP_OK(hipGetLastError());
    pst.end();
    if (p.ln_out) return launch_layernorm(p.out_f32, p.ln_gamma, p.ln_beta, p.ln_out, p.M, p.N, p.ln_eps, stream);
    return 0;
  }
  if (p.mode == EPI_HEADS) {
    const int64_t total_h = (int64_t)p.M * (p.N / 4);
    ProfScope psh("splitk_reduce", 0.0, (double)p.M * p.N * (4.0 * nsplit + 2.0), stream);
    SDMI_LAUNCH(splitk_reduce_heads_kernel, dim3((unsigned)((total_h + 255) / 256)), dim3(256), 0, stream, p, nsplit);
    SDMI_HIP_OK(hipGetLastError());
    return 0;
  }
  const int hw = p.Hout * p.Wout;
  if (p.gn_n > 0) SDMI_CHECK(hw % 32 == 0, "GroupNorm statistics need Hout*Wout % 32 == 0");
  const int rpb = reduce_rows_per_block(p);
  ProfScope ps2("splitk_reduce", 0.0, (double)p.M * p.N * 4.0 * (nsplit + 1), stream);
  SDMI_LAUNCH(splitk_reduce_kernel, dim3((unsigned)cdiv(p.N / 4, 8), (unsigned)cdiv(p.M, rpb)), dim3(256), 0, stream, p, nsplit,
                     rpb);
  SDMI_HIP_OK(hipGetLastError());
  ps2.end();
  if (p.ln_out) return launch_layernorm(p.out_f32, p.ln_gamma, p.ln_beta, p.ln_out, p.M, p.N, p.ln_eps, stream);
  return 0;
}

struct TileCfg { int bm, bn, wm, wn, ns; };
static const TileCfg kTiles[SDMI_NUM_TILES] = {
    {128, 128, 2, 2, 2},
    {128, 64, 2, 2, 2},
    {64, 64, 2, 2, 2},
    {256, 128, 4, 2, 2},
    {128, 64, 2, 2, 3},
    {64, 64, 2, 2, 3},
    {256, 128, 4, 2, 3},
    {128, 128, 2, 2, 3},
    {64, 128, 2, 2, 3},
    {128, 128, 4, 2, 3},
    {64, 64, 2, 2, 4},
    {128, 256, 2, 4, 2},
    {64, 256, 1, 4, 3},
    {256, 64, 4, 1, 3},
    {256, 64, 4, 2, 5},
    {256, 128, 4, 2, 3},
    {128, 64, 2, 2, 8},
    {128, 128, 2, 2, 5},
    {64, 64, 2, 2, 8},
    {64, 128, 2, 2, 6},
    {128, 64, 2, 2, 6},
    {128, 128, 4, 2, 4},
};
static inline bool tile_is_halo(int t) { return t >= 14 && t <= 17; }
static inline bool tile_tn_even(int t) { return (kTiles[t].bn / kTiles[t].wn / 32) % 2 == 0; }

static int launch_tile(int tile, const IGemmParams& p, bool dma, int splitk, hipStream_t stream) {
  if (p.split16) return launch_split16_tile(tile, p, splitk, stream);
  if (igemm_has_half(p)) {
    switch (tile) {
      case 0: case 1: case 2: case 3: case 4: case 5: return launch_generic_tile_h0(tile, p, dma, splitk, stream);
      case 6: case 7: case 8: case 9: case 10: return launch_generic_tile_h1(tile, p, dma, splitk, stream);
      case 11: case 12: case 13: case 18: case 19: case 20: case 21: return launch_generic_tile_h2(tile, p, dma, splitk, stream);
      default: break;
    }
  }
  switch (tile) {
    case 0: case 1: case 2: case 3: case 4: case 5: return launch_generic_tile_g0(tile, p, dma, splitk, stream);
    case 6: case 7: case 8: case 9: case 10: return launch_generic_tile_g1(tile, p, dma, splitk, stream);
    case 11: case 12: case 13: case 18: case 19: case 20: case 21: return launch_generic_tile_g2(tile, p, dma, splitk, stream);
    case 14: case 15: case 16: case 17: return launch_halo_tile(tile, p, splitk, stream);
    default: return fail("unknown igemm tile id");
  }
}

struct TuneKey {
  int M, N, K, ksize, stride, up, mode, splitk_req;
  bool operator<(const TuneKey& o) const {
    return std::tie(M, N, K, ksize, stride, up, mode, splitk_req) <
           std::tie(o.M, o.N, o.K, o.ksize, o.stride, o.up, o.mode, o.splitk_req);
  }
};
struct TuneChoice { int tile, splitk; double us; };
struct TuneRec { TuneKey key; int cand; hipEvent_t e0, e1; };

class Tuner {
 public:
  std::mutex mu;
  std::map<TuneKey, TuneChoice> table;
  bool loaded = false, collecting = false;
  int round = 0;
  std::vector<TuneRec> recs;
  std::map<TuneKey, std::vector<std::pair<TuneChoice, std::vector<float>>>> stats;
  std::vector<hipEvent_t> pool;

  static std::string default_path() {
    if (const char* e = getenv("SDMI_TUNE_FILE")) return e;
    Dl_info info;
    if (dladdr((const void*)&Tuner::default_path, &info) && info.dli_fname) {
      std::string so = info.dli_fname;
      const size_t k = so.find_last_of('/');
      return (k == std::string::npos ? std::string(".") : so.substr(0, k)) + "/tune_gfx950.txt";
    }
    return "tune_gfx950.txt";
  }
  void load_file(const std::string& path) {
    FILE* f = fopen(path.c_str(), "r");
    if (!f) return;
    char line[256];
    while (fgets(line, sizeof line, f)) {
      if (line[0] == '#') continue;
      TuneKey k; TuneChoice c; c.us = 0;
      if (sscanf(line, "%d %d %d %d %d %d %d %d %d %d %lf", &k.M, &k.N, &k.K, &k.ksize, &k.stride, &k.up, &k.mode,
                 &k.splitk_req, &c.tile, &c.splitk, &c.us) >= 10 && c.tile >= 0 && c.tile < SDMI_NUM_TILES && c.splitk >= 1 &&
          c.splitk <= 16)
        table[k] = c;
    }
    fclose(f);
  }
  void ensure_loaded() {
    if (loaded) return;
    loaded = true;
    if (env_int("SDMI_TUNE_DISABLE", 0)) return;
    load_file(default_path());
  }
  hipEvent_t ev() {
    if (!pool.empty()) { hipEvent_t e = pool.back(); pool.pop_back(); return e; }
    hipEvent_t e = nullptr;
    (void)hipEventCreate(&e);
    return e;
  }
};
static Tuner g_tuner;

static std::vector<TuneChoice> tune_candidates(const IGemmParams& p, bool can_split) {
  std::vector<TuneChoice> out;
  const int nkt = igemm_nkt(p);
  static const int splits[] = {1, 2, 3, 4, 5, 6, 8, 10, 12, 16};
  for (int t = 0; t < SDMI_NUM_TILES; ++t) {
    const TileCfg& c = kTiles[t];
    if (tile_is_halo(t) && !halo_supported(p, c.bm)) continue;
    if (p.split16 && !split16_tile_supported(t)) continue;
    if (!p.split16 && ((c.ns == 2 && t != 11 && !tile_is_halo(t)) || t == 12 || t == 13)) continue;
    if (p.mode == EPI_GEGLU && !tile_tn_even(t)) continue;
    if (p.lnp_out && (p.M % c.bm || p.N % c.bn || (p.Hout * p.Wout) % c.bm)) continue;
    const long blocks = (long)cdiv(p.M, c.bm) * cdiv(p.N, c.bn);
    if ((long)c.bm > 2L * p.M && c.bm > 64) continue;
    if ((long)c.bn > 2L * p.N && c.bn > 64) continue;
    for (int sk : splits) {
      if ((sk == 5 || sk == 10) && !tile_is_halo(t)) continue;
      if (sk > 1) {
        if (p.splitk != 0 || !can_split) break;
        if (nkt / sk < 4) break;
        if (tile_is_halo(t) && (nkt / 9) % sk != 0) continue;
        if (blocks * (sk / 2 + 1) > 1536) break;
        if (splitk_ws_need(p, c.bm, c.bn, sk) > p.splitk_ws_floats) break;
      }
      if (blocks * sk < 48 && sk < 16 && nkt / (sk * 2) >= 4 && can_split && p.splitk == 0) continue;
      out.push_back({t, p.splitk > 1 ? p.splitk : sk, 0.0});
      if (p.splitk != 0) break;
    }
  }
  if (out.empty()) out.push_back({5, p.splitk > 0 ? p.splitk : 1, 0.0});
  return out;
}

int tune_begin() {
  std::lock_guard<std::mutex> lk(g_tuner.mu);
  g_tuner.ensure_loaded();
  g_tuner.collecting = true; g_tuner.round = 0;
  g_tuner.recs.clear(); g_tuner.stats.clear();
  return 0;
}
int tune_round(int r) {
  std::lock_guard<std::mutex> lk(g_tuner.mu);
  g_tuner.round = r;
  return 0;
}
static int tune_drain() {
  for (auto& r : g_tuner.recs) {
    float ms = 0.f;
    SDMI_HIP_OK(hipEventSynchronize(r.e1));
    SDMI_HIP_OK(hipEventElapsedTime(&ms, r.e0, r.e1));
    auto& v = g_tuner.stats[r.key];
    if ((int)v.size() > r.cand) v[r.cand].second.push_back(ms * 1e3f);
    g_tuner.pool.push_back(r.e0); g_tuner.pool.push_back(r.e1);
  }
  g_tuner.recs.clear();
  return 0;
}
bool tune_collecting() { return g_tuner.collecting; }
static uint64_t g_tune_generation = 0;
uint64_t tune_generation() { return g_tune_generation; }
int tune_end(const char* path, int* n_keys) {
  std::lock_guard<std::mutex> lk(g_tuner.mu);
  if (!g_tuner.collecting) return fail("sdmi_tune_end without sdmi_tune_begin");
  if (tune_drain()) return -1;
  g_tuner.collecting = false;
  auto score = [](std::vector<float> v) -> double {
    if (v.empty()) return 1e30;
    std::sort(v.begin(), v.end());
    return v.size() % 2 ? v[v.size() / 2] : 0.5 * (v[v.size() / 2 - 1] + v[v.size() / 2]);
  };
  for (auto& kv : g_tuner.stats) {
    double best = 1e30; const TuneChoice* bc = nullptr;
    for (auto& c : kv.second) {
      const double sc = score(c.second);
      if (sc < best) { best = sc; bc = &c.first; }
    }
    if (bc) g_tuner.table[kv.first] = {bc->tile, bc->splitk, best};
  }
  if (n_keys) *n_keys = (int)g_tuner.stats.size();
  ++g_tune_generation;
  const std::string out = (path && *path) ? std::string(path) : Tuner::default_path();
  FILE* f = fopen(out.c_str(), "w");
  if (!f) return fail("cannot write the tuning table to " + out);
  fprintf(f, "# libsdmi igemm tuning table (gfx950), measured in situ by tools/tune.py -- M N K ksize stride up mode splitk_req tile splitk us\n");
  for (auto& kv : g_tuner.table) {
    const TuneKey& k = kv.first;
    fprintf(f, "%d %d %d %d %d %d %d %d %d %d %.2f\n", k.M, k.N, k.K, k.ksize, k.stride, k.up, k.mode, k.splitk_req, kv.second.tile,
            kv.second.splitk, kv.second.us);
  }
  fclose(f);
  return 0;
}
int tune_dump(std::string* out) {
  std::lock_guard<std::mutex> lk(g_tuner.mu);
  char buf[256];
  for (auto& kv : g_tuner.stats) {
    const TuneKey& k = kv.first;
    for (auto& c : kv.second) {
      if (c.second.empty()) continue;
      std::vector<float> v = c.second;
      std::sort(v.begin(), v.end());
      snprintf(buf, sizeof buf, "%d %d %d %d %d %d %d %d | %d %d %.2f %.2f %d\n", k.M, k.N, k.K, k.ksize, k.stride, k.up, k.mode,
               k.splitk_req, c.first.tile, c.first.splitk, (double)v[v.size() / 2], (double)v[0], (int)v.size());
      *out += buf;
    }
  }
  return 0;
}

int launch_igemm(const IGemmParams& p, const IGemmTune& tune, hipStream_t stream) {
  SDMI_CHECK(p.M > 0 && p.N > 0 && p.K > 0, "empty GEMM");
  SDMI_CHECK(p.ksize == 1 || p.ksize == 3, "ksize must be 1 or 3");
  const int Cin = p.c0 + p.c1 + p.c2;
  SDMI_CHECK(p.K == p.ksize * p.ksize * Cin, "K != ksize^2 * (c0 + c1 + c2)");
  SDMI_CHECK(p.c0 % BKH == 0 && p.c1 % BKH == 0 && p.c2 % BKH == 0 && p.c0 > 0, "channel counts of every A source must be multiples of 32");
  SDMI_CHECK((p.c2 == 0 || p.c1 > 0), "third A source without a second");
  SDMI_CHECK(p.lda0 % 8 == 0 && (p.a1 == nullptr || p.lda1 % 8 == 0), "A row pitch must be a multiple of 8 halves");
  SDMI_CHECK(p.zero_page != nullptr, "zero page missing");
  SDMI_CHECK(p.M == p.B * p.Hout * p.Wout, "M != B * Hout * Wout");
  SDMI_CHECK(p.c1 == 0 || p.a1 != nullptr, "second A source missing");
  SDMI_CHECK(p.c2 == 0 || (p.a2 != nullptr && p.lda2 % 8 == 0), "third A source missing");
  SDMI_CHECK((p.c1 == 0 || p.lda1 == p.lda0) && (p.c2 == 0 || p.lda2 == p.lda0), "all A sources must share one row pitch");
  SDMI_CHECK(!p.up || (p.ksize == 3 && p.stride == 1), "upsample folding needs a 3x3 stride-1 conv");
  if (p.mode == EPI_GEGLU) SDMI_CHECK(p.N % 64 == 0 && p.out_f16 != nullptr, "GEGLU needs N % 64 == 0 and an fp16 output");
  if (p.ln_out)
    SDMI_CHECK(p.mode == EPI_PLAIN && p.out_f32 && p.ldo == p.N && p.N % 4 == 0 && p.N <= 2560 && p.ln_gamma && p.ln_beta,
               "LayerNorm post-op needs plain mode, an fp32 output with ldo == N <= 2560, gamma and beta");
  if (p.out_lo) SDMI_CHECK(p.mode == EPI_PLAIN && p.ldo % 4 == 0, "out_lo needs plain mode");
  if (p.lnp_out || p.f16_scale)
    SDMI_CHECK(p.mode == EPI_PLAIN && p.out_f32 && p.out_f16 && !p.out_lo && !p.ln_out && p.N % 64 == 0 && p.M % 64 == 0 &&
                   (p.Hout * p.Wout) % 64 == 0 && p.splitk == 1 && epi_vec_ok(p),
               "LayerNorm row statistics: plain mode, fp32 + fp16 outputs, no split-K, M / N / rows per sample multiples of 64, 16-byte aligned rows");
  if (p.lnf_part)
    SDMI_CHECK(p.ksize == 1 && p.c1 == 0 && p.c2 == 0 && !p.split16 && p.lnf_npart * 32 == p.K && p.lnf_cs && p.lnf_d && !p.bias &&
                   p.splitk == 1 && p.lnf_npart <= 40,
               "LayerNorm-folding GEMM: dense, one source, K = 32 * lnf_npart <= 1280, column sums + offsets, no bias, no split-K");
  if (p.gn_n) {
    SDMI_CHECK(p.mode == EPI_PLAIN && p.gn_n <= 2 && (p.Hout * p.Wout) % 32 == 0, "GroupNorm statistics need plain mode and Hout*Wout % 32 == 0");
    SDMI_CHECK(p.N % 4 == 0, "GroupNorm statistics: N % 4 == 0");
    for (int t = 0; t < p.gn_n; ++t)
      SDMI_CHECK(p.gn_acc[t] && p.gn_cpg[t] >= 2 && (p.gn_cbase[t] + p.N + p.gn_cpg[t] - 1) / p.gn_cpg[t] <= 32, "bad GroupNorm statistics target");
  }
  if (p.mode == EPI_HEADS) SDMI_CHECK(p.segC > 0 && p.dh > 0 && p.N % p.segC == 0 && p.N / p.segC <= 3, "bad head scatter");

  SDMI_CHECK((int64_t)p.B * p.Hin * p.Win * p.lda0 * 2 + (int64_t)(p.Win + 1) * p.lda0 * 2 < ((int64_t)1 << 31) - 65536 &&
                 (int64_t)p.N * p.K * 2 < ((int64_t)1 << 31) - 65536,
             "tensor too large for 31-bit byte offsets (buffer addressing)");
  static const int env_dma = env_int("SDMI_IGEMM_DMA", 1);
  static const int env_tile = env_int("SDMI_IGEMM_TILE", -1);
  const bool dma = (tune.dma >= 0 ? tune.dma : env_dma) != 0;
  int tile = tune.tile >= 0 ? tune.tile : env_tile;
  SDMI_CHECK(tile < SDMI_NUM_TILES, "unknown igemm tile id");
  int splitk = p.splitk;
  const int nkt = igemm_nkt(p);
  static const int env_split = env_int("SDMI_SPLITK", -1);
  const bool can_split_plain = p.mode == EPI_PLAIN && p.splitk_ws && p.N % 4 == 0 && p.ldo % 4 == 0 &&
                               (p.residual == nullptr || p.ldr % 4 == 0);
  const bool can_split_heads = p.mode == EPI_HEADS && p.splitk_ws && p.dh % 4 == 0 && p.segC % 4 == 0;
  const bool can_split = can_split_plain || can_split_heads;
  if (env_split >= 0 && splitk == 0) splitk = env_split;

  hipEvent_t ev0 = nullptr, ev1 = nullptr;
  TuneKey tkey{p.M, p.N, nkt * BK, p.split16 ? 11 : p.ksize, p.stride, p.up, p.mode, splitk};
  int tcand = -1;
  if (tile < 0) {
    std::lock_guard<std::mutex> lk(g_tuner.mu);
    g_tuner.ensure_loaded();
    static const int only_ksize = env_int("SDMI_TUNE_ONLY_KSIZE", -1);
    if (g_tuner.collecting && (only_ksize < 0 || tkey.ksize == only_ksize)) {
      IGemmParams q = p; q.splitk = splitk;
      const std::vector<TuneChoice> cands = tune_candidates(q, can_split);
      auto& st = g_tuner.stats[tkey];
      if (st.empty()) for (auto& c : cands) st.push_back({c, {}});
      tcand = g_tuner.round % (int)cands.size();
      tile = cands[tcand].tile; splitk = cands[tcand].splitk;
      ev0 = g_tuner.ev(); ev1 = g_tuner.ev();
    } else {
      auto it = g_tuner.table.find(tkey);
      if (it != g_tuner.table.end()) {
        const int tt = it->second.tile, sk = it->second.splitk;
        const bool halo = tile_is_halo(tt);
        const bool ws_ok = sk == 1 || (can_split && splitk_ws_need(p, kTiles[tt].bm, kTiles[tt].bn, sk) <= p.splitk_ws_floats);
        const bool split_ok = splitk != 0 ? (sk == splitk && ws_ok)
                                          : (sk == 1 || (ws_ok && nkt / sk >= 4 && (halo || (sk != 5 && sk != 10)) &&
                                                         (!halo || (nkt / 9) % sk == 0)));
        if (split_ok && (p.mode != EPI_GEGLU || tile_tn_even(tt)) && (!halo || halo_supported(p, kTiles[tt].bm)) &&
            (!p.split16 || split16_tile_supported(tt))) {
          tile = tt; splitk = sk;
        }
      }
    }
  }
  if (p.mode == EPI_GEGLU && tile >= 0 && !tile_tn_even(tile)) tile = 0;
  if (p.split16) {
    if (tile >= 0) SDMI_CHECK(split16_tile_supported(tile), "split-fp16 GEMM: tile id without an instantiation");
    else tile = 5;
  }
  if (tile < 0) {
    const double gflop = 2.0 * p.M * (double)p.N * p.K * 1e-9;
    if (p.mode == EPI_GEGLU) tile = 0;
    else if (p.mode == EPI_HEADS) tile = 2;
    else tile = gflop >= 25.0 ? 3 : 5;
  }
  if (p.lnp_out) {
    const int hw = p.Hout * p.Wout;
    if (p.M % kTiles[tile].bm || p.N % kTiles[tile].bn || hw % kTiles[tile].bm || (p.split16 && !split16_tile_supported(tile))) tile = 5;
  }
  if (splitk <= 0) {
    splitk = 1;
    if (can_split) {
      const long blocks = (long)cdiv(p.M, kTiles[tile].bm) * cdiv(p.N, kTiles[tile].bn);
      const long want = (kTiles[tile].wm * kTiles[tile].wn == 8) ? 160 : 512;
      while (blocks * splitk < want && nkt / (splitk * 2) >= 8 && splitk < 16 &&
             splitk_ws_need(p, kTiles[tile].bm, kTiles[tile].bn, splitk * 2) <= p.splitk_ws_floats)
        splitk *= 2;
    }
  }
  if (splitk > 1) {
    SDMI_CHECK(can_split, "split-K needs plain or head-scatter mode, a slab workspace and N / ldo / ldr multiples of 4");
    SDMI_CHECK(splitk_ws_need(p, kTiles[tile].bm, kTiles[tile].bn, splitk) <= p.splitk_ws_floats, "split-K workspace too small");
  }
  if (ev0) SDMI_HIP_OK(hipEventRecord(ev0, stream));
#ifdef SDMI_IGEMM_TIMING
  static const char* dbg_path = getenv("SDMI_IGEMM_TIMING");
  static const int dbg_abl = env_int("SDMI_EPI_ABL", 0);
  static long long* dbg_buf = nullptr;
  constexpr int DBG_WG = 16384;
  IGemmParams pd = p;
  pd.dbg_abl = dbg_abl;
  if (dbg_path) {
    if (!dbg_buf) SDMI_HIP_OK(hipMalloc((void**)&dbg_buf, 6 * DBG_WG * sizeof(long long)));
    SDMI_HIP_OK(hipMemsetAsync(dbg_buf, 0, 6 * DBG_WG * sizeof(long long), stream));
    pd.dbg_times = dbg_buf;
  }
  const int rc = launch_tile(tile, pd, dma, splitk, stream);
  if (dbg_path && pd.dbg_times && rc == 0) {
    SDMI_HIP_OK(hipStreamSynchronize(stream));
    std::vector<long long> h(6 * DBG_WG);
    SDMI_HIP_OK(hipMemcpy(h.data(), dbg_buf, h.size() * sizeof(long long), hipMemcpyDeviceToHost));
    std::vector<long long> pro, loop, epi, sto, start;
    long long tmin = 0, tmax = 0;
    for (int b = 0; b < DBG_WG; ++b) {
      const long long* d = &h[6 * b];
      if (d[4] == 0) continue;
      pro.push_back(d[1] - d[0]); loop.push_back(d[2] - d[1]); epi.push_back(d[4] - d[2]);
      sto.push_back(d[3] ? d[3] - d[2] : d[4] - d[2]);
      if (start.empty() || d[0] < tmin) tmin = d[0];
      if (d[4] > tmax) tmax = d[4];
      start.push_back(d[0]);
    }
    if (!pro.empty()) {
      auto med = [](std::vector<long long>& v) { std::sort(v.begin(), v.end()); return v[v.size() / 2]; };
      auto mx = [](std::vector<long long>& v) { return *std::max_element(v.begin(), v.end()); };
      long long late = 0;
      for (long long t : start) late = std::max(late, t - tmin);
      if (FILE* f = fopen(dbg_path, "a")) {
        const int nkt_split = (p.K / BK + std::max(splitk, 1) - 1) / std::max(splitk, 1);
        fprintf(f, "M%d N%d K%d k%d mode%d tile%d split%d res%d gn%d blocks%zu k-tiles/block %d | shader cycles: span %lld last-start %lld | median prologue %lld loop %lld epilogue %lld (stores %lld) | max loop %lld max epi %lld | loop cycles per k-tile %.1f\n",
                p.M, p.N, p.K, p.ksize, p.mode, tile, splitk, p.residual ? 1 : 0, p.gn_n, pro.size(), nkt_split, tmax - tmin, late, med(pro), med(loop),
                med(epi), med(sto), mx(loop), mx(epi), (double)med(loop) / nkt_split);
        fclose(f);
// ... 27 lines not shown
```

### stable-diffusion_amd/csrc/unet.cpp

```cpp
#include "unet.h"

extern "C" char** environ;
#include "prof.h"
#include "split16.h"

#include <math.h>
#include <stdio.h>
#include <string.h>

#include <algorithm>

namespace sdmi {

static bool in_list(const int* v, int n, int x) {
  for (int i = 0; i < n; ++i)
    if (v[i] == x) return true;
  return false;
}

thread_local Tape* g_tape_rec = nullptr;

namespace {
uint64_t sdmi_env_hash() {
  uint64_t h = 1469598103934665603ull;
// ... 200 lines not shown
      }
      case L_ATTN_LEGACY: {
        const int64_t C = ci;
        const bool pq = L.p1x1;
        store_.expect(p + ".norm.weight", {C}, W_F32, &L.f32[0]);
        store_.expect(p + ".norm.bias", {C}, W_F32, &L.f32[1]);
        WeightSlot& qkv = store_.expect(p + ".qkv.weight", {3 * C, C, 1}, W_QKV_LEGACY, &L.w16[0]);
        qkv.heads = L.heads; qkv.split = pq;
        store_.expect(p + ".qkv.bias", {3 * C}, W_QKV_LEGACY_B, &L.f32[2]).heads = L.heads;
        store_.expect(p + ".proj_out.weight", {C, C, 1}, full() ? W_SPLIT3 : W_ROWS16, &L.w16[1]);
        store_.expect(p + ".proj_out.bias", {C}, W_F32, &L.f32[3]);
        break;
      }
      case L_DOWN:
        store_.expect(p + ".op.weight", {co, ci, 3, 3}, full() ? W_CONV_SPLIT3 : W_CONV, &L.w16[0]);
        store_.expect(p + ".op.bias", {co}, W_F32, &L.f32[0]);
        break;
      case L_UP:
        store_.expect(p + ".conv.weight", {co, ci, 3, 3}, full() ? W_CONV_SPLIT3 : W_CONV, &L.w16[0]);
        store_.expect(p + ".conv.bias", {co}, W_F32, &L.f32[0]);
        break;
    }
    return 0;
  });
  store_.expect("out.0.weight", {mc}, W_F32, &out_gamma_);
  store_.expect("out.0.bias", {mc}, W_F32, &out_beta_);
  store_.expect("out.2.weight", {c.out_channels, mc, 3, 3}, W_CONV_OUT, &out_w_);
  store_.expect("out.2.bias", {c.out_channels}, W_F32, &out_b_);
  return 0;
}

UNet::~UNet() {
  if (emb_tab_) (void)hipFree(emb_tab_);
  if (emb_tab_tdev_) (void)hipFree(emb_tab_tdev_);
  for_each_layer([](Layer& L) -> int {
    for (auto& T : L.tb) {
      if (T.ck) (void)hipFree(T.ck);
      if (T.cvt) (void)hipFree(T.cvt);
      if (T.ck_lo) (void)hipFree(T.ck_lo);
      if (T.cvt_lo) (void)hipFree(T.cvt_lo);
    }
    return 0;
  });
}

int UNet::set_weight(const char* key, const float* ptr, const int64_t* shape, int ndim, hipStream_t stream) {
  if (int rc = store_.set(key, ptr, shape, ndim, stream)) return rc;
  ++weights_gen_;
  finalized_ = false;
  ctx_valid_ = false;
  drop_timestep_table();
  return 0;
}

int UNet::finalize() {
  if (const WeightSlot* m = store_.missing()) return fail("weight not set: " + m->key);
  if (store_.zero_page()) return -1;
  if (reserve_ctx_cache(8, 77)) return -1;
  {
    SDMI_HIP_OK(hipDeviceSynchronize());
    if (for_each_layer([&](Layer& L) -> int {
      if (L.kind != L_ATTN || full()) return 0;
      const int C = L.cin;
      for (auto& T : L.tb) {
        const int n_[3] = {3 * C, C, 8 * C};
        const f16* w_[3] = {T.wqkv, T.wq2, T.wgg};
        const float* b_[3] = {nullptr, nullptr, T.bgg};
        for (int i = 0; i < 3; ++i) {
          if (store_.alloc((void**)&T.lnf[2 * i], (size_t)n_[i] * sizeof(float)) || store_.alloc((void**)&T.lnf[2 * i + 1], (size_t)n_[i] * sizeof(float)))
            return -1;
          if (launch_ln_fold_prep(w_[i], n_[i], C, C, T.ln[2 * i], T.ln[2 * i + 1], b_[i], T.lnf[2 * i], T.lnf[2 * i + 1], nullptr)) return -1;
        }
        if (ff_tail_supported(C, 32, 32)) {
          if (store_.alloc((void**)&T.lnf_csd, (size_t)16 * C * sizeof(float))) return -1;
          for (int h = 0; h < 4; ++h) {
            SDMI_HIP_OK(hipMemcpyAsync(T.lnf_csd + (size_t)h * 4 * C, T.lnf[4] + (size_t)h * 2 * C, (size_t)2 * C * sizeof(float), hipMemcpyDeviceToDevice, nullptr));
            SDMI_HIP_OK(hipMemcpyAsync(T.lnf_csd + (size_t)h * 4 * C + 2 * C, T.lnf[5] + (size_t)h * 2 * C, (size_t)2 * C * sizeof(float), hipMemcpyDeviceToDevice, nullptr));
          }
        }
      }
      return 0;
    })) return -1;
    SDMI_HIP_OK(hipDeviceSynchronize());
  }
  ++weights_gen_;
  finalized_ = true;
  return 0;
}

namespace {
struct PackedHeader {
  char magic[8];
  int32_t abi, precise_1x1, n_buffers, reserved;
  sdmi_unet_cfg cfg;
  int64_t total_bytes;
};
constexpr int64_t PK_ALIGN = 256;
constexpr int PK_NHC_SHIFT = 16;
constexpr int32_t PK_NHC_MASK = 0xfff << PK_NHC_SHIFT;
constexpr int32_t PK_FULL = 4;
}

int UNet::packed_layout(std::vector<std::pair<void**, size_t>>* bufs, int64_t* total) const {
  int64_t off = (int64_t)round_up((int64_t)sizeof(PackedHeader), PK_ALIGN);
  for (const auto& b : store_.buffers()) {
    if (bufs) bufs->push_back(b);
    off += (int64_t)round_up((int64_t)b.second, PK_ALIGN);
  }
  *total = off;
  return 0;
}

int UNet::export_packed(void* host_buf, int64_t bytes, hipStream_t stream) {
  SDMI_CHECK(finalized_, "export needs a finalized handle");
  std::vector<std::pair<void**, size_t>> bufs;
  int64_t total = 0;
  packed_layout(&bufs, &total);
  SDMI_CHECK(host_buf && bytes >= total, "packed buffer too small: need " + std::to_string(total) + " bytes");
  PackedHeader h{};
  memcpy(h.magic, "SDMIPK01", 8);
  h.abi = SDMI_ABI_VERSION; h.precise_1x1 = precise_1x1_ ? 1 : 0; h.n_buffers = (int32_t)bufs.size(); h.cfg = cfg_;
  h.reserved = (precise_kv_ ? 1 : 0) | (precise_last_res_ ? 2 : 0) | (precise_1x1_max_ds_ << 8);
  h.reserved |= (ext_.attention_block << 4) | (ext_.resblock_updown << 5) | ((scale_shift_ ? 1 : 0) << 6);
  h.reserved |= num_head_channels_ << PK_NHC_SHIFT;
  if (full()) h.reserved |= PK_FULL;
  h.total_bytes = total;
  memcpy(host_buf, &h, sizeof(h));
  int64_t off = (int64_t)round_up((int64_t)sizeof(PackedHeader), PK_ALIGN);
  for (auto& b : bufs) {
    SDMI_HIP_OK(hipMemcpyAsync((char*)host_buf + off, *b.first, b.second, hipMemcpyDeviceToHost, stream));
    off += (int64_t)round_up((int64_t)b.second, PK_ALIGN);
  }
  SDMI_HIP_OK(hipStreamSynchronize(stream));
  return 0;
}

int UNet::import_packed(const void* host_buf, int64_t bytes, hipStream_t stream) {
  SDMI_CHECK(host_buf && bytes >= (int64_t)sizeof(PackedHeader), "packed blob truncated");
  PackedHeader h;
  memcpy(&h, host_buf, sizeof(h));
  SDMI_CHECK(memcmp(h.magic, "SDMIPK01", 8) == 0, "not a libsdmi packed-weight blob");
  SDMI_CHECK(h.abi == SDMI_ABI_VERSION, "packed blob was written by a different ABI version: repack it");
  SDMI_CHECK(memcmp(&h.cfg, &cfg_, sizeof(cfg_)) == 0, "packed blob was written for a different UNet configuration");
  SDMI_CHECK(((h.reserved & PK_FULL) != 0) == full(), std::string("packed blob was written by a ") +
             ((h.reserved & PK_FULL) ? "full" : "mixed") + "-precision UNet handle and cannot be imported into a " + (full() ? "full" : "mixed") +
             "-precision one: repack it with a handle of this precision");
  SDMI_CHECK((h.precise_1x1 != 0) == precise_1x1_, "packed blob was written with a different precision allocation (split-fp16 1x1 convs)");
  SDMI_CHECK((h.reserved & (7 << 4)) == ((ext_.attention_block << 4) | (ext_.resblock_updown << 5) | ((scale_shift_ ? 1 : 0) << 6)),
             "packed blob was written for a different UNet family (attention_block / resblock_updown / scale-shift norm)");
  SDMI_CHECK(((h.reserved & PK_NHC_MASK) >> PK_NHC_SHIFT) == num_head_channels_,
             "packed blob was written for num_head_channels " + std::to_string((h.reserved & PK_NHC_MASK) >> PK_NHC_SHIFT) + ", this handle has " +
             std::to_string(num_head_channels_) + ": repack it");
  SDMI_CHECK((h.reserved & ~PK_FULL & ~(7 << 4) & ~PK_NHC_MASK) == ((precise_kv_ ? 1 : 0) | (precise_last_res_ ? 2 : 0) | (precise_1x1_max_ds_ << 8)),
             "packed blob was written with a different precision allocation (context K / V, last ResBlock, 1x1 conv levels)");
  std::vector<std::pair<void**, size_t>> bufs;
  int64_t total = 0;
  packed_layout(&bufs, &total);
  SDMI_CHECK(h.n_buffers == (int32_t)bufs.size() && h.total_bytes == total && bytes >= total, "packed blob truncated or inconsistent");
  int64_t off = (int64_t)round_up((int64_t)sizeof(PackedHeader), PK_ALIGN);
  for (auto& b : bufs) {
    if (store_.alloc(b.first, b.second)) return -1;
    SDMI_HIP_OK(hipMemcpyAsync(*b.first, (const char*)host_buf + off, b.second, hipMemcpyHostToDevice, stream));
    off += (int64_t)round_up((int64_t)b.second, PK_ALIGN);
  }
  SDMI_HIP_OK(hipStreamSynchronize(stream));
  store_.mark_all_set();
  ctx_valid_ = false;
  drop_timestep_table();
  return finalize();
}

struct Fwd : FwdBase {
  UNet* u; int Lctx;
  bool ln_fold_on = false;
  bool ff_tail_on = false;
  bool st_head_on = false;
  bool st_mid_on = false;
  bool st_tail_on = false;
  bool st_mid_ctx_on = false;
  bool ctx1_on = false;
  bool gn_conv_on = false;
  float* emb_all = nullptr;
  int emb_ld = 0;
  bool emb_caller = false;
  const f16* ctx16 = nullptr;
  const f16* ctx16_lo = nullptr;

  Act res_block(Layer& L, const Act& x0, const Act* x1) {
    const int H = x0.H, W = x0.W, M = B * H * W;
    const int Cin = x0.C + (x1 ? x1->C : 0), Cout = L.cout;
    if (Cin != L.cin) { ok(fail("res block channel mismatch at " + L.prefix)); }
    if (Cin == Cout && x1) ok(fail("identity skip with a concatenated input at " + L.prefix));
    const size_t mark = scratch.off;
    f16* raw = (Cin != Cout) ? S<f16>((size_t)M * Cin) : nullptr;
    const bool p1 = L.p1x1;
    const bool p3 = L.precise3;
    f16* raw_lo = (Cin != Cout && p1) ? S<f16>((size_t)M * Cin) : nullptr;
    float* h = S<float>((size_t)M * Cout);
    Act out = make_act(P<float>((size_t)M * Cout), Cout, H, W, true);
    Act hact = make_act(h, Cout, H, W, true);
    f16* a2 = nullptr;
    int& gn2_applied = u->gn2_applied_;
    gn2_applied = 0;
    const bool ss = u->scale_shift_;
    const float* const film = ss ? emb_all + L.emb_off : nullptr;
    const bool gc1 = gn_conv_on && !ss && !p3 && Cin == Cout && gn_conv3_supported(B, H, W, x0.C, x1 ? x1->C : 0, Cout);
    const bool gc2 = gn_conv_on && !ss && !p3 && gn_conv3_supported(B, H, W, Cout, 0, Cout);
    auto gn_conv = [&](const Act& a0, const Act* a1, const float* gamma, const float* beta, const f16* w, IGemmParams& e) {
      GnConvParams g = GnConvParams();
      g.gn_acc = groupnorm(a0, a1, gamma, beta, 1e-5f, 1, nullptr, nullptr, nullptr, nullptr, nullptr, true);
      g.x0 = a0.p; g.c0 = a0.C; g.x1 = a1 ? a1->p : nullptr; g.c1 = a1 ? a1->C : 0;
      g.gn_gamma = gamma; g.gn_beta = beta; g.gn_eps = 1e-5f; g.w = w; g.epi = e;
      if (!dry && !rc) ok(launch_gn_conv3(g, s));
    };
    if (gc1) {
      IGemmParams p = conv3(nullptr, Cin, H, W, H, W, 1, 0, L.w16[0], Cout);
      p.bias = L.f32[2]; p.rowvec = emb_all + L.emb_off; p.ld_rowvec = emb_ld;
      p.out_f32 = h; p.ldo = Cout;
      attach_gn_targets(p, hact);
      TapeCaller tc(Tape::R_EMB, emb_caller ? p.rowvec : nullptr);
      gn_conv(x0, x1, L.f32[0], L.f32[1], L.w16[0], p);
    } else {
      f16* a = S<f16>((size_t)M * Cin);
      f16* a_lo = p3 ? S<f16>((size_t)M * Cin) : nullptr;
      groupnorm(x0, x1, L.f32[0], L.f32[1], 1e-5f, 1, a, nullptr, raw, a_lo, raw_lo);
      IGemmParams p = conv3(a, Cin, H, W, H, W, 1, 0, L.w16[0], Cout);
      if (p3) split3(p, a, a_lo, Cin);
      p.bias = L.f32[2];
      if (!ss) { p.rowvec = emb_all + L.emb_off; p.ld_rowvec = emb_ld; }
      p.out_f32 = h; p.ldo = Cout;
      attach_gn_targets(p, hact);
      if (!gc2 && !p3 && !ss) {
        a2 = S<f16>((size_t)M * Cout);
        p.pgn_gamma = L.f32[3]; p.pgn_beta = L.f32[4]; p.pgn_eps = 1e-5f; p.pgn_silu = 1; p.pgn_out = a2; p.pgn_applied = &gn2_applied;
      }
      TapeCaller tc(Tape::R_EMB, emb_caller ? p.rowvec : nullptr);
      gemm(p);
    }
    const float* residual = x0.p;
    if (Cin != Cout) {
      IGemmParams p = dense1x1(raw, raw_lo, M, Cin, L.w16[2], Cout, H * W, p1);
      p.bias = L.f32[6]; p.out_f32 = out.p; p.ldo = Cout;
      gemm(p);
      residual = out.p;
    }
    if (gc2) {
      IGemmParams p = conv3(nullptr, Cout, H, W, H, W, 1, 0, L.w16[1], Cout);
      p.bias = L.f32[5]; p.residual = residual; p.ldr = Cout; p.out_f32 = out.p; p.ldo = Cout;
      attach_gn_targets(p, out);
      attach_f16_copy(p, out);
      gn_conv(hact, nullptr, L.f32[3], L.f32[4], L.w16[1], p);
    } else {
      f16* a2_lo = nullptr;
      if (p3) { a2 = S<f16>((size_t)M * Cout); a2_lo = S<f16>((size_t)M * Cout); }
      if (ss && !a2) a2 = S<f16>((size_t)M * Cout);
      {
        TapeCaller tc(Tape::R_EMB, emb_caller ? film : nullptr);
        groupnorm(hact, nullptr, L.f32[3], L.f32[4], 1e-5f, 1, a2, nullptr, nullptr, a2_lo, nullptr, false, gn2_applied != 0, film, emb_ld);
      }
      IGemmParams p = conv3(a2, Cout, H, W, H, W, 1, 0, L.w16[1], Cout);
      if (p3) split3(p, a2, a2_lo, Cout);
      p.bias = L.f32[5]; p.residual = residual; p.ldr = Cout; p.out_f32 = out.p; p.ldo = Cout;
      attach_gn_targets(p, out);
      attach_f16_copy(p, out);
      gemm(p);
    }
    scratch.off = mark;
    return out;
  }

  void context_kv(Layer& L, int d) {
    TBlock& T = L.tb[d];
    const int C = L.cin, Lp = (int)round_up(Lctx, 8);
    const int CD = u->cfg_.context_dim;
    IGemmParams p = dense(ctx16, B * Lctx, CD, T.wkv2, 2 * C, Lctx);
    if (ctx16_lo) split3(p, ctx16, ctx16_lo, CD);
    if (u->full()) {
      const size_t mark = scratch.off;
      float* kv = S<float>((size_t)B * Lctx * 2 * C);
      p.out_f32 = kv; p.ldo = 2 * C;
      gemm(p);
      if (!dry && !rc) ok(launch_split_heads(kv, 2 * C, 0, T.ck, T.ck_lo, 0, B, Lctx, Lp, L.heads, L.dh, s));
      if (!dry && !rc) ok(launch_split_heads(kv, 2 * C, C, T.cvt, T.cvt_lo, 1, B, Lctx, Lp, L.heads, L.dh, s));
      scratch.off = mark;
      return;
    }
    p.mode = EPI_HEADS; p.seg_dst[0] = T.ck; p.seg_dst[1] = T.cvt; p.seg_kind[0] = 0; p.seg_kind[1] = 1;
    p.heads = L.heads; p.dh = L.dh; p.ntok = Lctx; p.ntok_pad = Lp; p.segC = C; p.splitk = 1;
    if (!dry && !rc && Lp != Lctx) {
      hipError_t e = memset_async(T.cvt, 0, (size_t)B * C * Lp * sizeof(f16), s);
      if (e != hipSuccess) ok(fail(std::string("hipMemsetAsync: ") + hipGetErrorString(e)));
    }
    gemm(p);
  }

  Act attn_block_full(Layer& L, const Act& x) {
    const int H = x.H, W = x.W, N = H * W, M = B * N, C = L.cin;
    const int Np = (int)round_up(N, 8), Lp = (int)round_up(Lctx, 8);
    const float scale = 1.0f / sqrtf((float)L.dh);
    const size_t mark = scratch.off;
    f16* a = S<f16>((size_t)M * C); f16* a_lo = S<f16>((size_t)M * C);
    float* t = S<float>((size_t)M * C);
    float* y = S<float>((size_t)M * 8 * C);
    f16* q = S<f16>((size_t)M * C); f16* q_lo = S<f16>((size_t)M * C);
    f16* k = S<f16>((size_t)M * C); f16* k_lo = S<f16>((size_t)M * C);
    f16* vt = S<f16>((size_t)B * C * Np); f16* vt_lo = S<f16>((size_t)B * C * Np);
    f16* gg = S<f16>((size_t)M * 4 * C); f16* gg_lo = S<f16>((size_t)M * 4 * C);
    auto linear = [&](const f16* hi, const f16* lo, int K, const f16* w, int n_out, const float* bias, float* out, bool residual) {
      IGemmParams p = dense1x1(hi, lo, M, K, w, n_out, N, true);
      p.bias = bias; p.out_f32 = out; p.ldo = n_out;
      if (residual) { p.residual = out; p.ldr = n_out; }
      gemm(p);
    };
    auto layernorm = [&](const float* gamma, const float* beta) {
      if (!dry && !rc) ok(launch_layernorm_split(t, gamma, beta, a, a_lo, M, C, 1e-5f, s));
    };
    auto heads = [&](const float* src, int ld, int col0, f16* dst, f16* dst_lo, int kind) {
      if (!dry && !rc) ok(launch_split_heads(src, ld, col0, dst, dst_lo, kind, B, N, Np, L.heads, L.dh, s));
    };
    auto attend = [&](const f16* kk, const f16* kk_lo, const f16* v, const f16* v_lo, int nkv, int nkv_pad) {
      AttnSplitParams p = AttnSplitParams();
      p.q = q; p.q_lo = q_lo; p.k = kk; p.k_lo = kk_lo; p.vt = v; p.vt_lo = v_lo; p.out = a; p.out_lo = a_lo;
      p.BH = B * L.heads; p.heads = L.heads; p.nq = N; p.nkv = nkv; p.nkv_pad = nkv_pad; p.d = L.dh; p.scale = scale;
      if (!dry && !rc) ok(launch_attention_split16(p, s));
    };
    groupnorm(x, nullptr, L.f32[0], L.f32[1], 1e-6f, 0, a, nullptr, nullptr, a_lo, nullptr);
    linear(a, a_lo, C, L.w16[0], C, L.f32[2], t, false);
    for (auto& T : L.tb) {
      layernorm(T.ln[0], T.ln[1]);
      linear(a, a_lo, C, T.wqkv, 3 * C, nullptr, y, false);
      heads(y, 3 * C, 0, q, q_lo, 0); heads(y, 3 * C, C, k, k_lo, 0); heads(y, 3 * C, 2 * C, vt, vt_lo, 1);
      attend(k, k_lo, vt, vt_lo, N, Np);
      linear(a, a_lo, C, T.wo1, C, T.bo1, t, true);
      layernorm(T.ln[2], T.ln[3]);
      if (ctx16) context_kv(L, (int)(&T - L.tb.data()));
      linear(a, a_lo, C, T.wq2, C, nullptr, y, false);
      heads(y, C, 0, q, q_lo, 0);
      attend(T.ck, T.ck_lo, T.cvt, T.cvt_lo, Lctx, Lp);
      linear(a, a_lo, C, T.wo2, C, T.bo2, t, true);
      layernorm(T.ln[4], T.ln[5]);
      linear(a, a_lo, C, T.wgg, 8 * C, T.bgg, y, false);
      if (!dry && !rc) ok(launch_geglu_split(y, M, 4 * C, gg, gg_lo, s));
      linear(gg, gg_lo, 4 * C, T.wff2, C, T.bff2, t, true);
    }
    if (!dry && !rc) ok(launch_cast_f16(t, a, a_lo, (int64_t)M * C, s));
// ... 388 lines not shown
  else SDMI_CHECK(H >= 1 && W >= 1 && Lctx == 0 && ctx == nullptr && !ctx_only,
                  "bad shape: this UNet has no cross-attention (AttentionBlocks): pass ctx = NULL and Lctx = 0");
  const int down = 1 << (cfg_.n_levels - 1);
  if (ext_.resblock_updown)
    SDMI_CHECK(H % down == 0 && W % down == 0, "latent H and W must be multiples of " + std::to_string(down) +
               " for resblock_updown (the down ResBlocks' avg_pool2d rounds down, the skip concat needs the sizes back)");
  SDMI_CHECK(H % down == 0 && W % down == 0, "H and W must be divisible by 2^(levels-1) (the UNet's skip concat requires it)");

  const int hint_row = emb_hint_row_;
  if (!dry && !ctx_only) emb_hint_row_ = -1;

  const char* e_rp = getenv("SDMI_REPLAY"); const char* e_rv = getenv("SDMI_REPLAY_VERIFY");
  const bool replay_on = !(e_rp && atoi(e_rp) == 0);
  const bool replay_verify = e_rv && atoi(e_rv) != 0;
  const bool hinted = t_i64 != nullptr && hint_row >= 0 && hint_row < (int)emb_tab_t_.size();
  auto in_ws = [&](const void* p, size_t bytes) {
    return p && (uintptr_t)p < (uintptr_t)workspace + (uint64_t)ws_bytes && (uintptr_t)workspace < (uintptr_t)p + bytes;
  };
  const size_t img = (size_t)B * H * W * sizeof(float);
  const bool tape_ok = replay_on && !dry && !ctx_only && !prof_enabled() && !tune_collecting() && !range_check_enabled() &&
                       workspace != nullptr && (t_i64 || t_f32) && !in_ws(x, img * cfg_.in_channels) && !in_ws(eps_out, img * cfg_.out_channels) &&
                       !in_ws(t_i64 ? (const void*)t_i64 : t_f32, (size_t)B * (t_i64 ? 8 : 4)) &&
                       !in_ws(ctx, (size_t)B * Lctx * cfg_.context_dim * sizeof(float));
  TapeKey tkey;
  uintptr_t caller[Tape::R_COUNT] = {0, 0, 0, 0, 0};
  Tape* rec = nullptr;
  std::unique_ptr<Tape> verify_against;
  if (tape_ok) {
    tkey.B = B; tkey.H = H; tkey.W = W; tkey.Lctx = Lctx; tkey.mode = hinted ? 0 : (t_i64 ? 1 : 2);
    tkey.ws = workspace; tkey.ws_bytes = ws_bytes; tkey.have_ctx = ctx != nullptr;
    tkey.env = sdmi_env_hash() ^ (tune_generation() * 0x9e3779b97f4a7c15ull); tkey.weights_gen = weights_gen_; tkey.ctx_gen = ctx_gen_;
    auto low4 = [](const void* p, int shift) { return (unsigned)((uintptr_t)p & 15) << shift; };
    tkey.align = low4(x, 0) | low4(eps_out, 4) | low4(ctx, 8) | low4(t_i64 ? (const void*)t_i64 : t_f32, 12);
    caller[Tape::R_X] = (uintptr_t)x; caller[Tape::R_OUT] = (uintptr_t)eps_out;
    caller[Tape::R_T] = hinted ? 0 : (t_i64 ? (uintptr_t)t_i64 : (uintptr_t)t_f32);
    caller[Tape::R_CTX] = (uintptr_t)ctx;
    caller[Tape::R_EMB] = hinted ? (uintptr_t)(emb_tab_ + (size_t)hint_row * emb_total_) : 0;
    for (size_t i = 0; i < tapes_.size(); ++i) {
      if (!(tapes_[i].first == tkey)) continue;
      std::unique_ptr<Tape> hit = std::move(tapes_[i].second);
      tapes_.erase(tapes_.begin() + (long)i);
      SDMI_CHECK(finalized_, "sdmi_unet_finalize() has not succeeded yet");
      if (ensure_ctx_cache(B, Lctx, false)) return -1;
      if (!ctx && has_ctx()) SDMI_CHECK(ctx_valid_, "ctx == NULL but no cached context for this (B, Lctx); call sdmi_unet_cache_context first");
      hit->retarget(caller);
      if (replay_verify) { verify_against = std::move(hit); break; }
      const int e = hit->replay(stream);
      const bool sets = hit->sets_ctx_valid;
      const int64_t need = hit->bytes_needed;
      tapes_.emplace_back(tkey, std::move(hit));
      if (e) return fail(std::string("launch tape replay: ") + hipGetErrorString((hipError_t)e));
      if (sets) ctx_valid_ = true;
      if (bytes_needed) *bytes_needed = need;
      ++tape_hits_;
      return 0;
    }
  }
  std::unique_ptr<Tape> fresh;
  if (tape_ok) {
    fresh.reset(new Tape());
    memcpy(fresh->caller, caller, sizeof(caller));
    rec = fresh.get();
  }

  Fwd f;
  f.u = this; f.s = stream; f.dry = dry; f.B = B; f.Lctx = Lctx; f.zero = store_.zero(); f.precise_1x1 = precise_1x1_;
  {
    const char* e_fold = getenv("SDMI_LN_FOLD"); const char* e_vec = getenv("SDMI_EPI_VEC");
    f.ln_fold_on = (e_fold ? atoi(e_fold) != 0 : ln_fold_) && !(e_vec && atoi(e_vec) == 0);
    const char* e_ff = getenv("SDMI_FF_TAIL");
    f.ff_tail_on = e_ff ? atoi(e_ff) != 0 : ff_tail_;
    const char* e_sh = getenv("SDMI_ST_HEAD");
    f.st_head_on = e_sh ? atoi(e_sh) != 0 : st_head_;
    const char* e_sm = getenv("SDMI_ST_MID");
    f.st_mid_on = e_sm ? atoi(e_sm) != 0 : st_head_;
    const char* e_st = getenv("SDMI_ST_TAIL");
    f.st_tail_on = e_st ? atoi(e_st) != 0 : ff_tail_;
    const char* e_mc = getenv("SDMI_ST_MID_CTX");
    f.st_mid_ctx_on = e_mc ? atoi(e_mc) != 0 : st_head_;
    const char* e_c1 = getenv("SDMI_CTX1");
    f.ctx1_on = !(e_c1 && atoi(e_c1) == 0);
    const char* e_gc = getenv("SDMI_GN_CONV");
    f.gn_conv_on = e_gc ? atoi(e_gc) != 0 : false;
    if (full()) {
      f.ln_fold_on = f.ff_tail_on = f.st_head_on = f.st_mid_on = f.st_tail_on = f.st_mid_ctx_on = f.gn_conv_on = false;
    }
  }
  int64_t persist_bytes = 0, scratch_bytes = 0;
  for (int pass = 0; pass < 2; ++pass) {
    const bool d = (pass == 0) ? true : false;
    if (pass == 1 && dry) break;
    f.dry = d; f.rc = 0;
    f.n_acts = 0;
    TapeRecGuard tape_guard(d ? nullptr : rec);
    f.plan = fuse_gn_stats_ ? &gn_plan_ : nullptr;
    if (d) gn_plan_.clear();
    f.persist = Arena(); f.scratch = Arena();
    f.persist.dry = f.scratch.dry = d;
    if (!d) {
      SDMI_CHECK(persist_bytes + scratch_bytes <= ws_bytes, "workspace too small: need " +
                 std::to_string(persist_bytes + scratch_bytes) + " bytes, got " + std::to_string(ws_bytes));
      SDMI_CHECK(workspace != nullptr, "workspace is NULL");
      f.persist.base = (char*)workspace; f.persist.cap = (size_t)persist_bytes;
      f.scratch.base = (char*)workspace + persist_bytes; f.scratch.cap = (size_t)scratch_bytes;
      if (ensure_ctx_cache(B, Lctx, ctx_only)) return -1;
    }
    const int mc = cfg_.model_channels;
    if (f.begin_pass((int64_t)12 << 20)) return -1;
    f16* ctx16 = f.P<f16>((size_t)B * Lctx * cfg_.context_dim);
    f16* ctx16_lo = precise_kv_ ? f.P<f16>((size_t)B * Lctx * cfg_.context_dim) : nullptr;
    const bool have_ctx = has_ctx() && ((ctx != nullptr) || d);
    if (!has_ctx()) {
      f.ctx16 = nullptr; f.ctx16_lo = nullptr;
    } else if (have_ctx) {
      if (!d) {
        TapeCaller tc(Tape::R_CTX, ctx);
        int r = launch_cast_f16(ctx, ctx16, ctx16_lo, (int64_t)B * Lctx * cfg_.context_dim, stream);
        if (r) return r;
      }
      f.ctx16 = ctx16; f.ctx16_lo = ctx16_lo;
    } else {
      SDMI_CHECK(ctx_valid_, "ctx == NULL but no cached context for this (B, Lctx); call sdmi_unet_cache_context first");
      f.ctx16 = nullptr; f.ctx16_lo = nullptr;
    }
    if (ctx_only) {
      for_each_layer([&](Layer& L) -> int {
        if (L.kind == L_ATTN) for (int dd = 0; dd < (int)L.tb.size(); ++dd) f.context_kv(L, dd);
        return 0;
      });
    } else {
      float* temb = f.P<float>((size_t)B * mc);
      float* e1 = f.P<float>((size_t)B * te_);
      float* emb = f.P<float>((size_t)B * te_);
      f.emb_all = f.P<float>((size_t)B * emb_total_);
      f.emb_ld = emb_total_;
      if (!d && t_i64 != nullptr && hint_row >= 0 && hint_row < (int)emb_tab_t_.size()) {
        f.emb_all = emb_tab_ + (size_t)hint_row * emb_total_;
        f.emb_ld = 0;
        f.emb_caller = true;
      } else if (!d) {
        int r;
        {
          TapeCaller tc(Tape::R_T, t_i64 ? (const void*)t_i64 : t_f32);
          r = launch_timestep_embedding(t_i64, t_f32, temb, B, mc, stream);
        }
        if (!r) r = launch_small_linear(temb, mc, te_w0_, te_b0_, e1, te_, B, te_, mc, 0, stream);
        if (!r) r = launch_small_linear(e1, te_, te_w2_, te_b2_, emb, te_, B, te_, te_, 1, stream);
        if (!r) r = launch_small_linear(emb, te_, emb_w_, emb_b_, f.emb_all, emb_total_, B, emb_total_, te_, 1, stream);
        if (r) return r;
      }
      std::vector<Act> hs;
      Act h;
      {
        Layer& L = input_blocks_[0][0];
        const char* e_cis = getenv("SDMI_CONV_IN_STATS");
        h = f.make_act(f.P<float>((size_t)B * H * W * mc), mc, H, W, (H * W) % 16 == 0 && !(e_cis && atoi(e_cis) == 0));
        IGemmParams st = IGemmParams();
        f.attach_gn_targets(st, h);
        if (!d) {
          TapeCaller tc(Tape::R_X, x);
          int r = launch_conv_in(x, L.w32[0], L.f32[0], h.p, B, cfg_.in_channels, H, W, mc, stream, st.gn_n, st.gn_acc, st.gn_cpg, st.gn_cbase);
          if (r) return r;
        }
        hs.push_back(h);
      }
      for (size_t bi = 1; bi < input_blocks_.size(); ++bi) {
// ... 60 lines not shown
```

### stable-diffusion_amd/csrc/unet.h

```cpp
#pragma once
#include <stdlib.h>

#include <memory>
#include <string>
#include <utility>
#include <vector>

#include "../../include/sdmi.h"
#include "common.h"
#include "weights.h"

namespace sdmi {

struct Arena {
  char* base = nullptr; size_t cap = 0, off = 0, peak = 0; bool dry = false; bool overflow = false;
  void* alloc(size_t bytes) {
    const size_t a = (off + 255) & ~(size_t)255;
    off = a + bytes;
    peak = std::max(peak, off);
    if (dry) return (void*)(uintptr_t)(a + 4096);
    if (off > cap) { overflow = true; return base; }
    return base + a;
  }
};
// ... 91 lines not shown
    IGemmParams p = IGemmParams();
    p.a0 = a; p.c0 = K; p.lda0 = K;
    p.B = M / rows_per_batch; p.Hin = p.Hout = rows_per_batch; p.Win = p.Wout = 1;
    p.ksize = 1; p.w = w; p.M = M; p.N = N; p.K = K; p.splitk = 0;
    return p;
  }
  IGemmParams conv3(const f16* a, int C, int Hin, int Win, int Hout, int Wout, int stride, int up, const f16* w, int N) {
    IGemmParams p = IGemmParams();
    p.a0 = a; p.c0 = C; p.lda0 = C;
    p.B = B; p.Hin = Hin; p.Win = Win; p.Hout = Hout; p.Wout = Wout;
    p.ksize = 3; p.stride = stride; p.up = up; p.w = w; p.M = B * Hout * Wout; p.N = N; p.K = 9 * C; p.splitk = 0;
    return p;
  }
  static void split3(IGemmParams& p, const f16* hi, const f16* lo, int C) {
    p.a0 = hi; p.c0 = C; p.lda0 = C; p.a1 = lo; p.c1 = C; p.lda1 = C; p.a2 = hi; p.c2 = C; p.lda2 = C;
    p.k_alg = p.ksize * p.ksize * C; p.K = 3 * p.k_alg;
  }
  IGemmParams dense1x1(const f16* hi, const f16* lo, int M, int K, const f16* w, int N, int rows_per_batch, bool precise) {
    IGemmParams p = dense(hi, M, K, w, N, rows_per_batch);
    if (precise) {
      static const bool family = !(getenv("SDMI_SPLIT16_KERNEL") && atoi(getenv("SDMI_SPLIT16_KERNEL")) == 0);
      if (family && K % 32 == 0) { p.a1 = lo; p.lda1 = K; p.split16 = 1; p.ldw = 3 * K; }
      else split3(p, hi, lo, K);
    }
    return p;
  }
  long long* groupnorm(const Act& x0, const Act* x1, const float* gamma, const float* beta, float eps, int silu, f16* o16,
                       float* o32, f16* raw, f16* o16_lo = nullptr, f16* raw_lo = nullptr, bool stats_only = false,
                       bool already_applied = false, const float* film = nullptr, int film_ld = 0) {
    GroupNormParams g = GroupNormParams();
    g.film = film; g.film_ld = film_ld;
    g.x0 = x0.p; g.c0 = x0.C;
    if (x1) { g.x1 = x1->p; g.c1 = x1->C; }
    g.B = B; g.HW = x0.H * x0.W; g.gamma = gamma; g.beta = beta; g.eps = eps; g.silu = silu;
    g.out_f16 = o16; g.out_f32 = o32; g.raw_f16 = raw; g.out_lo = o16_lo; g.raw_lo = raw_lo;
    g.stats_only = stats_only ? 1 : 0;
    const int idx = gn_calls;
    g.acc = next_gn_acc();
    if (plan) {
      const int cpg = (g.c0 + g.c1) / 32;
      if (dry) {
        const bool f = x0.stats && (!x1 || x1->stats) && x0.id >= 0 && (!x1 || x1->id >= 0);
        if ((int)plan->fused.size() <= idx) plan->fused.resize(idx + 1, 0);
        plan->fused[idx] = f ? 1 : 0;
        if (f) {
          plan->targets[x0.id].push_back({idx, 0, cpg});
          if (x1) plan->targets[x1->id].push_back({idx, g.c0, cpg});
        }
      } else {
        g.skip_stats = (idx < (int)plan->fused.size() && plan->fused[idx]) ? 1 : 0;
      }
    }
    if (!dry && !rc && !(stats_only && g.skip_stats) && !already_applied) ok(launch_groupnorm(g, s));
    return g.acc;
  }
};

enum LayerKind { L_CONV_IN, L_RES, L_ATTN, L_DOWN, L_UP, L_ATTN_LEGACY };

struct TBlock {
  f16* wqkv = nullptr;
  f16* wo1 = nullptr; float* bo1 = nullptr;
  f16* wq2 = nullptr;
  f16* wkv2 = nullptr;
  f16* wo2 = nullptr; float* bo2 = nullptr;
  f16* wgg = nullptr; float* bgg = nullptr;
  f16* wff2 = nullptr; float* bff2 = nullptr;
  float* ln[6] = {nullptr, nullptr, nullptr, nullptr, nullptr, nullptr};
  f16* ck = nullptr; f16* cvt = nullptr;
  f16* ck_lo = nullptr; f16* cvt_lo = nullptr;
  float* lnf[6] = {nullptr, nullptr, nullptr, nullptr, nullptr, nullptr};
  float* lnf_csd = nullptr;
};

struct Layer {
  LayerKind kind = L_RES;
  std::string prefix;
  int cin = 0, cout = 0, heads = 0, dh = 0, emb_off = 0, attn_index = -1;
  int updown = 0;
  bool p1x1 = true, precise3 = false;
  f16* w16[3] = {nullptr, nullptr, nullptr};
  float* w32[1] = {nullptr};
  float* f32[7] = {nullptr, nullptr, nullptr, nullptr, nullptr, nullptr, nullptr};
  std::vector<TBlock> tb;
};

class UNet {
 public:
  UNet() = default;
  ~UNet();
  UNet(const UNet&) = delete;
  UNet& operator=(const UNet&) = delete;

  int build(const sdmi_unet_cfg& cfg, int precision = SDMI_PRECISION_MIXED, const sdmi_unet_ext* ext = nullptr, unsigned flags = 0);
  int set_weight(const char* key, const float* ptr, const int64_t* shape, int ndim, hipStream_t stream);
  int finalize();
  int packed_layout(std::vector<std::pair<void**, size_t>>* bufs, int64_t* total) const;
  int export_packed(void* host_buf, int64_t bytes, hipStream_t stream);
  int import_packed(const void* host_buf, int64_t bytes, hipStream_t stream);
  int run(const float* x, const int64_t* t_i64, const float* t_f32, const float* ctx, float* eps_out, int B, int H, int W,
          int Lctx, void* workspace, int64_t ws_bytes, hipStream_t stream, bool dry, bool ctx_only, int64_t* bytes_needed);

  int cache_timesteps(const int64_t* t_host, int n, hipStream_t stream);
  int reserve_ctx_cache(int B, int Lctx);
  int hint_timestep(int64_t t);

  const WeightStore& weights() const { return store_; }

  sdmi_unet_cfg cfg_{};
  sdmi_unet_ext ext_{};
  bool has_ctx() const { return ext_.attention_block == 0; }
  bool scale_shift_ = false;
  int num_head_channels_ = 0;
  int precision_ = SDMI_PRECISION_MIXED;
  bool full() const { return precision_ == SDMI_PRECISION_FULL; }
  int te_ = 0, emb_total_ = 0, n_attn_ = 0;
  bool precise_1x1_ = true;
  bool precise_last_res_ = true;
  int precise_1x1_max_ds_ = 4;
  bool precise_kv_ = true;

 private:
  friend struct Fwd;
  template <class F> int for_each_layer(F&& fn) {
    for (auto& blk : input_blocks_) for (auto& L : blk) if (int r = fn(L)) return r;
    for (auto& L : middle_) if (int r = fn(L)) return r;
    for (auto& blk : output_blocks_) for (auto& L : blk) if (int r = fn(L)) return r;
    return 0;
  }
  int ensure_ctx_cache(int B, int Lctx, bool may_grow);
  GnPlan gn_plan_;
  bool fuse_gn_stats_ = true;
  bool ln_fold_ = true; int ln_fold_min_rows_ = 512;
  bool ff_tail_ = true;
  bool st_head_ = true;

  struct TapeKey {
    int B = 0, H = 0, W = 0, Lctx = 0, mode = 0;
    const void* ws = nullptr; int64_t ws_bytes = 0; bool have_ctx = false;
    uint64_t env = 0, weights_gen = 0, ctx_gen = 0;
    unsigned align = 0;
    bool operator==(const TapeKey& o) const {
      return B == o.B && H == o.H && W == o.W && Lctx == o.Lctx && mode == o.mode && ws == o.ws && ws_bytes == o.ws_bytes &&
             have_ctx == o.have_ctx && env == o.env && weights_gen == o.weights_gen && ctx_gen == o.ctx_gen && align == o.align;
    }
  };
  std::vector<std::pair<TapeKey, std::unique_ptr<Tape>>> tapes_;
  static constexpr size_t kMaxTapes = 12;
  uint64_t weights_gen_ = 0, ctx_gen_ = 0;
  int gn2_applied_ = 0;
 public:
  uint64_t tape_hits_ = 0, tape_records_ = 0;
 private:

  std::vector<std::vector<Layer>> input_blocks_, output_blocks_;
  std::vector<Layer> middle_;
  WeightStore store_;
  float *te_w0_ = nullptr, *te_b0_ = nullptr, *te_w2_ = nullptr, *te_b2_ = nullptr;
  float *emb_w_ = nullptr, *emb_b_ = nullptr;
  float *out_gamma_ = nullptr, *out_beta_ = nullptr, *out_w_ = nullptr, *out_b_ = nullptr;
  bool finalized_ = false;
  int ctx_B_ = 0, ctx_L_ = 0; bool ctx_valid_ = false;
  int64_t ctx_cap_ = 0;
  float* emb_tab_ = nullptr; size_t emb_tab_floats_ = 0;
  int64_t* emb_tab_tdev_ = nullptr; size_t emb_tab_tcap_ = 0;
  std::vector<int64_t> emb_tab_t_;
  std::vector<int64_t> emb_tab_src_;
  int emb_hint_row_ = -1;
  void drop_timestep_table() { emb_tab_t_.clear(); emb_hint_row_ = -1; }
};

}
```

Baseline: 3.623.

## Fold ResBlock 1x1 skip projection into the second conv3x3 as a tail K-phase

Measured after the change: 3.674, median of 6. 1.01x the previous value.

```diff
diff --git a/include/sdmi.h b/include/sdmi.h
--- a/include/sdmi.h
+++ b/include/sdmi.h
@@ -63,6 +63,7 @@
 int sdmi_unet_cache_timesteps(sdmi_unet* h, const int64_t* t_host, int n, void* stream);
 int sdmi_unet_hint_timestep(sdmi_unet* h, int64_t t);
 int sdmi_unet_tape_stats(sdmi_unet* h, int64_t* replayed, int64_t* recorded);
+int sdmi_unet_skip_fold_plan(sdmi_unet* h, int B, int H, int W, int Lctx, int32_t* folded, int cap);
 
 int sdmi_unet_forward(sdmi_unet* h, const float* x, const int64_t* t_i64, const float* t_f32, const float* ctx,
                       float* eps_out, int B, int H, int W, int Lctx, void* workspace, int64_t workspace_bytes,
@@ -178,6 +179,9 @@
   void* out_lo;
 } sdmi_igemm_desc;
 int sdmi_k_igemm(const sdmi_igemm_desc* d, void* stream);
+int sdmi_k_igemm_tail(const sdmi_igemm_desc* d, const void* t0, const void* t1, const void* t2, int tail_c, int tail_ld, const void* tail_w,
+                      int tail_kt, void* stream);
+int sdmi_k_tail_split_range(int nkt, int nsplit, int split, int* begin, int* end);
 int sdmi_k_ff_tail(const sdmi_igemm_desc* proj_out, const void* ln_f16, const float* lnp, float ln_eps, const float* csd,
                    const void* wgg_f16, const void* wff2_f16, const float* bff2, const float* t, void* stream);
 int sdmi_k_st_tail(const sdmi_igemm_desc* proj_out, const void* a_f16, const void* wo_f16, const float* bo, float* t, const float* ln_gamma,
@@ -246,6 +250,7 @@
 int sdmi_tune_round(int r);
 int sdmi_tune_end(const char* path, int* n_keys);
 int sdmi_tune_dump(char* buf, int buflen);
+int sdmi_tune_lookup(int M, int N, int K, int ksize, int stride, int up, int mode, int splitk_req, int kt, int* tile, int* splitk);
 int sdmi_profile_begin(void);
 int sdmi_profile_end(char* json_buf, int json_buf_len);
 int sdmi_k_prefetch_lines(const void* ptr, int64_t bytes, void* stream);
diff --git a/stable-diffusion_amd/_lib.py b/stable-diffusion_amd/_lib.py
--- a/stable-diffusion_amd/_lib.py
+++ b/stable-diffusion_amd/_lib.py
@@ -126,6 +126,10 @@
     'sdmi_bert_forward': (C.c_int, [c_ptr, c_ptr, c_ptr, C.c_int, C.c_int, c_ptr, C.c_int64, c_ptr]),
     'sdmi_has_experiments': (C.c_int, []),
     'sdmi_k_igemm': (C.c_int, [C.POINTER(IGemmDesc), c_ptr]),
+    'sdmi_k_igemm_tail': (C.c_int, [C.POINTER(IGemmDesc), c_ptr, c_ptr, c_ptr, C.c_int, C.c_int, c_ptr, C.c_int, c_ptr]),
+    'sdmi_k_tail_split_range': (C.c_int, [C.c_int, C.c_int, C.c_int, C.POINTER(C.c_int), C.POINTER(C.c_int)]),
+    'sdmi_tune_lookup': (C.c_int, [C.c_int] * 9 + [C.POINTER(C.c_int), C.POINTER(C.c_int)]),
+    'sdmi_unet_skip_fold_plan': (C.c_int, [c_ptr, C.c_int, C.c_int, C.c_int, C.c_int, C.POINTER(C.c_int32), C.c_int]),
     'sdmi_k_ff_tail': (C.c_int, [C.POINTER(IGemmDesc), c_ptr, c_ptr, C.c_float, c_ptr, c_ptr, c_ptr, c_ptr, c_ptr, c_ptr]),
     'sdmi_k_gn_conv3': (C.c_int, [C.POINTER(IGemmDesc), c_ptr, c_ptr, C.c_int, C.c_int, c_ptr, C.c_int64, c_ptr, c_ptr, C.c_float, c_ptr]),
     'sdmi_k_st_mid_ctx': (C.c_int, [c_ptr, c_ptr, c_ptr, c_ptr, c_ptr, C.c_float, c_ptr, c_ptr, c_ptr, c_ptr, c_ptr, C.c_int, C.c_int, C.c_float, c_ptr,
diff --git a/stable-diffusion_amd/csrc/api.cpp b/stable-diffusion_amd/csrc/api.cpp
--- a/stable-diffusion_amd/csrc/api.cpp
+++ b/stable-diffusion_amd/csrc/api.cpp
@@ -353,6 +353,33 @@
   IGemmTune t; t.tile = d->tile; t.dma = d->dma;
   return launch_igemm(p, t, (hipStream_t)stream);
 }
+int sdmi_k_igemm_tail(const sdmi_igemm_desc* d, const void* t0, const void* t1, const void* t2, int tail_c, int tail_ld, const void* tail_w,
+                      int tail_kt, void* stream) {
+  SDMI_CHECK(d, "null descriptor");
+  IGemmParams p = IGemmParams();
+  if (igemm_params_of(d, p)) return -1;
+  p.tail_a0 = (const f16*)t0; p.tail_a1 = (const f16*)t1; p.tail_a2 = (const f16*)t2;
+  p.tail_c = tail_c; p.tail_ld = tail_ld; p.tail_w = (const f16*)tail_w; p.tail_kt = tail_kt;
+  IGemmTune t; t.tile = d->tile; t.dma = d->dma;
+  return launch_igemm(p, t, (hipStream_t)stream);
+}
+int sdmi_k_tail_split_range(int nkt, int nsplit, int split, int* begin, int* end) {
+  SDMI_CHECK(begin && end && nkt >= 0 && nsplit >= 1 && split >= 0 && split < nsplit, "bad arguments");
+  tail_split_range(nkt, nsplit, split, begin, end);
+  return 0;
+}
+int sdmi_tune_lookup(int M, int N, int K, int ksize, int stride, int up, int mode, int splitk_req, int kt, int* tile, int* splitk) {
+  SDMI_CHECK(tile && splitk, "null argument");
+  return tune_lookup(M, N, K, ksize, stride, up, mode, splitk_req, kt, tile, splitk);
+}
+int sdmi_unet_skip_fold_plan(sdmi_unet* h, int B, int H, int W, int Lctx, int32_t* folded, int cap) {
+  SDMI_CHECK(h && (folded || cap == 0), "null argument");
+  int64_t need = 0;
+  if (h->impl.run(nullptr, nullptr, nullptr, nullptr, nullptr, B, H, W, Lctx, nullptr, 0, nullptr, true, false, &need)) return -1;
+  const std::vector<int>& plan = h->impl.skip_fold_plan_;
+  for (int i = 0; i < (int)plan.size() && i < cap; ++i) folded[i] = plan[i];
+  return (int)plan.size();
+}
 int sdmi_k_ff_tail(const sdmi_igemm_desc* proj_out, const void* ln_f16, const float* lnp, float ln_eps, const float* csd,
                    const void* wgg_f16, const void* wff2_f16, const float* bff2, const float* t, void* stream) {
   SDMI_CHECK(proj_out, "null descriptor");
diff --git a/stable-diffusion_amd/csrc/common.h b/stable-diffusion_amd/csrc/common.h
--- a/stable-diffusion_amd/csrc/common.h
+++ b/stable-diffusion_amd/csrc/common.h
@@ -173,7 +173,15 @@
   unsigned long long magic_cpg_in = 0;
   int halo_thi = 0, halo_ipt = 1, log2_tpi = 30;
   unsigned long long magic_hpi = 0;
-};
+  const f16* tail_a0 = nullptr; const f16* tail_a1 = nullptr; const f16* tail_a2 = nullptr;
+  int tail_c = 0, tail_ld = 0;
+  const f16* tail_w = nullptr;
+  int tail_kt = 0;
+};
+__host__ __device__ static inline void tail_split_range(int nkt, int nsplit, int split, int* begin, int* end) {
+  *begin = (int)(((long long)split * nkt) / nsplit);
+  *end = (int)(((long long)(split + 1) * nkt) / nsplit);
+}
 
 constexpr int SDMI_NUM_TILES = 22;
 struct IGemmTune {
@@ -182,6 +190,8 @@
 };
 
 int launch_igemm(const IGemmParams& p, const IGemmTune& tune, hipStream_t stream);
+bool igemm_plans_halo(const IGemmParams& p);
+int tune_lookup(int M, int N, int K, int ksize, int stride, int up, int mode, int splitk_req, int kt, int* tile, int* splitk);
 bool range_check_enabled();
 uint64_t tune_generation();
 bool tune_collecting();
diff --git a/stable-diffusion_amd/csrc/conv3halo.hip b/stable-diffusion_amd/csrc/conv3halo.hip
--- a/stable-diffusion_amd/csrc/conv3halo.hip
+++ b/stable-diffusion_amd/csrc/conv3halo.hip
@@ -3,7 +3,7 @@
 namespace sdmi {
 namespace {
 
-template <int BM, int BN, int WARPS_M, int WARPS_N, int NS>
+template <int BM, int BN, int WARPS_M, int WARPS_N, int NS, bool TAIL = false>
 __global__ void __launch_bounds__(WARPS_M* WARPS_N * 64) conv3halo_kernel(const IGemmParams p, const int tiles_m,
                                                                            const int tiles_n, const int chunks_per_split) {
 #if defined(__HIP_DEVICE_COMPILE__)
@@ -219,6 +219,97 @@
     }
   }
   wait_vmcnt<0>();
+  if constexpr (TAIL) {
+    int t_begin, t_end;
+    tail_split_range(p.tail_kt / BK, p.splitk, split, &t_begin, &t_end);
+    if (t_begin < t_end) {
+      constexpr int A_PASSES = BM / RPP;
+      constexpr int STAGE_T = (BM + BN) * 128;
+      constexpr int NS_T = LDS_BYTES / STAGE_T < 4 ? LDS_BYTES / STAGE_T : 4;
+      constexpr int LPT = A_PASSES + PB;
+      constexpr int PPU = (LPT + U - 2) / (U - 1);
+      static_assert(A_PASSES >= 1 && NS_T >= 3 && NS_T * STAGE_T <= LDS_BYTES && LPT * (NS_T - 2) <= 48, "tail ring");
+      asm volatile("s_waitcnt lgkmcnt(0)\n\ts_barrier" ::: "memory");
+      int ta_off[A_PASSES], tb_off[PB];
+#pragma unroll
+      for (int i = 0; i < A_PASSES; ++i) ta_off[i] = (min(m0 + i * RPP + lrow, p.M - 1) * p.tail_ld + gch * 8) * 2;
+#pragma unroll
+      for (int i = 0; i < PB; ++i) tb_off[i] = (min(n0 + i * RPP + lrow, p.N - 1) * p.tail_kt + gch * 8) * 2;
+      const __amdgpu_buffer_rsrc_t rsrc_tw = __builtin_amdgcn_make_buffer_rsrc((void*)p.tail_w, 0, OOB, 0x00020000);
+      const char* const srcT0 = (const char*)p.tail_a0; const char* const srcT1 = (const char*)p.tail_a1;
+      const char* const srcT2 = (const char*)p.tail_a2;
+      const int tc = p.tail_c;
+      int ld_kt = t_begin;
+      const int tc2 = 2 * tc;
+      struct TailCursor { __amdgpu_buffer_rsrc_t rsrc_a; int a_soff, b_soff; unsigned lds; };
+      auto next_tile = [&](int stage) {
+        TailCursor c;
+        const int k0 = ld_kt * BK;
+        const char* src; int coff;
+        if (k0 < tc) { src = srcT0; coff = k0; }
+        else if (k0 < tc2) { src = srcT1; coff = k0 - tc; }
+        else { src = srcT2; coff = k0 - tc2; }
+        c.rsrc_a = __builtin_amdgcn_make_buffer_rsrc((void*)src, 0, OOB, 0x00020000);
+        c.a_soff = coff * 2; c.b_soff = k0 * 2; c.lds = stage * STAGE_T;
+        if (ld_kt + 1 < t_end) ++ld_kt;
+        return c;
+      };
+      auto issue_piece = [&](const TailCursor& c, int q) {
+        const unsigned row0 = (q < A_PASSES ? q * RPP : BM + (q - A_PASSES) * RPP) + wave_u * 8;
+        auto dst = (__attribute__((address_space(3))) void*)(smem + c.lds + row0 * 128);
+        if (q < A_PASSES) __builtin_amdgcn_raw_ptr_buffer_load_lds(c.rsrc_a, dst, 16, ta_off[q], c.a_soff, 0, 0);
+        else __builtin_amdgcn_raw_ptr_buffer_load_lds(rsrc_tw, dst, 16, tb_off[q - A_PASSES], c.b_soff, 0, SDMI_W_AUX);
+      };
+      const int ta_lds = (wm * WTM + l31) * 128, tb_lds = BM * 128 + (wn * WTN + l31) * 128;
+      auto read_tail = [&](int stage, int ks, f16x8 (&a)[TM], f16x8 (&b)[TN]) {
+        const unsigned char* st = smem + stage * STAGE_T + (((ks * 2 + lg) ^ rsw) << 4);
+#pragma unroll
+        for (int i = 0; i < TM; ++i) a[i] = *(const f16x8*)(st + ta_lds + i * 32 * 128);
+#pragma unroll
+        for (int j = 0; j < TN; ++j) b[j] = *(const f16x8*)(st + tb_lds + j * 32 * 128);
+      };
+#pragma unroll
+      for (int s2 = 0; s2 < NS_T - 1; ++s2) {
+        const TailCursor c = next_tile(s2);
+#pragma unroll
+        for (int q = 0; q < LPT; ++q) issue_piece(c, q);
+      }
+      wait_vmcnt<LPT*(NS_T - 2)>();
+      asm volatile("s_waitcnt lgkmcnt(0)\n\ts_barrier" ::: "memory");
+#pragma unroll
+      for (int g = 0; g < G; ++g) read_tail(0, g, fa[0][g], fb[0][g]);
+      int tcur = 0, tnxt = NS_T - 1;
+      for (int kt = t_begin; kt < t_end; ++kt) {
+        const TailCursor c = next_tile(tnxt);
+        const int tcur1 = (tcur + 1 == NS_T) ? 0 : tcur + 1;
+#pragma unroll
+        for (int u = 0; u < U; ++u) {
+          if (u + 1 < U) {
+#pragma unroll
+            for (int g = 0; g < G; ++g) read_tail(tcur, (u + 1) * G + g, fa[(u + 1) & 1][g], fb[(u + 1) & 1][g]);
+#pragma unroll
+            for (int q = u * PPU; q < (u + 1) * PPU && q < LPT; ++q) issue_piece(c, q);
+          } else {
+            wait_vmcnt<LPT*(NS_T - 2)>();
+            asm volatile("s_waitcnt lgkmcnt(0)\n\ts_barrier" ::: "memory");
+#pragma unroll
+            for (int g = 0; g < G; ++g) read_tail(tcur1, g, fa[0][g], fb[0][g]);
+          }
+#pragma unroll
+          for (int g = 0; g < G; ++g) mfma_step(fa[u & 1][g], fb[u & 1][g]);
+          __builtin_amdgcn_sched_group_barrier(0x100, G * (TM + TN), 0);
+#pragma unroll
+          for (int e = 0; e < MPU; ++e) {
+            __builtin_amdgcn_sched_group_barrier(0x008, 1, 0);
+            if (u + 1 < U && e < PPU && u * PPU + e < LPT) __builtin_amdgcn_sched_group_barrier(0x010, 1, 0);
+          }
+        }
+        tcur = tcur1;
+        tnxt = (tnxt + 1 == NS_T) ? 0 : tnxt + 1;
+      }
+      wait_vmcnt<0>();
+    }
+  }
   SDMI_STAMP(dbg_t2);
   igemm_epilogue<BM, BN, WARPS_M, WARPS_N, LDS_BYTES>(p, acc, m0, n0, split, tile_m, tile_n, smem);
 #ifdef SDMI_IGEMM_TIMING
@@ -246,6 +337,15 @@
 template <int BM, int BN, int WARPS_M, int WARPS_N, int NS>
 int launch_halo_cfg(const IGemmParams& p, int splitk, hipStream_t stream) {
   SDMI_CHECK(halo_supported(p, BM), "halo-staged conv tile requested for an unsupported shape");
+  if (p.tail_kt) {
+    const int nsrc = p.tail_c > 0 ? p.tail_kt / p.tail_c : 0;
+    SDMI_CHECK(p.tail_c > 0 && p.tail_c % BK == 0 && nsrc >= 1 && nsrc <= 3 && nsrc * p.tail_c == p.tail_kt && p.tail_w && p.tail_a0 &&
+                   (nsrc < 2 || p.tail_a1) && (nsrc < 3 || p.tail_a2) && p.tail_ld >= p.tail_c && p.tail_ld % 8 == 0,
+               "1x1 tail: one to three sources of tail_c % 64 == 0 channels, tail_kt = sources * tail_c, pitch >= tail_c and % 8 == 0");
+    SDMI_CHECK((int64_t)p.M * p.tail_ld * 2 < ((int64_t)1 << 31) - 65536 && (int64_t)p.N * p.tail_kt * 2 < ((int64_t)1 << 31) - 65536,
+               "1x1 tail: tensor too large for 31-bit byte offsets (buffer addressing)");
+    SDMI_CHECK(p.mode == EPI_PLAIN && p.M % BM == 0, "1x1 tail: plain mode, whole row tiles");
+  }
   const int tiles_m = cdiv(p.M, BM), tiles_n = cdiv(p.N, BN);
   const int nch = (p.c0 + p.c1 + p.c2) / BK;
   const int chunks_per_split = cdiv(nch, splitk);
@@ -279,13 +379,15 @@
   std::string pname = std::string("conv3halo_") + std::to_string(BM) + "x" + std::to_string(BN) + "w" +
                       std::to_string(WARPS_M * WARPS_N) + "s" + std::to_string(NS);
   if (by_shape && prof_enabled())
-    pname += "_M" + std::to_string(p.M) + "_N" + std::to_string(p.N) + "_K" + std::to_string(p.K) + "_s" + std::to_string(nsplit);
+    pname += "_M" + std::to_string(p.M) + "_N" + std::to_string(p.N) + "_K" + std::to_string(p.K) + "_s" + std::to_string(nsplit) +
+             (p.tail_kt ? "_t" + std::to_string(p.tail_kt) : std::string());
   const double src_pix = (double)p.B * p.Hin * p.Win;
-  ProfScope ps(pname.c_str(), 2.0 * p.M * (double)p.N * p.K,
+  ProfScope ps(pname.c_str(), 2.0 * p.M * (double)p.N * (p.K + (p.tail_kt ? p.tail_c : 0)),
                src_pix * (p.c0 + p.c1) * 2.0 + (double)p.N * p.K * 2.0 + (double)p.M * p.N * ((p.out_f32 ? 4.0 : 0.0) + (p.out_f16 ? 2.0 : 0.0)) +
-                   (p.residual ? (double)p.M * p.N * 4.0 : 0.0),
+                   (p.residual ? (double)p.M * p.N * 4.0 : 0.0) + (p.tail_kt ? ((double)p.M + p.N) * p.tail_c * 2.0 : 0.0),
                stream);
-  SDMI_LAUNCH((conv3halo_kernel<BM, BN, WARPS_M, WARPS_N, NS>), grid, block, 0, stream, q, tiles_m, tiles_n, chunks_per_split);
+  if (p.tail_kt) SDMI_LAUNCH((conv3halo_kernel<BM, BN, WARPS_M, WARPS_N, NS, true>), grid, block, 0, stream, q, tiles_m, tiles_n, chunks_per_split);
+  else SDMI_LAUNCH((conv3halo_kernel<BM, BN, WARPS_M, WARPS_N, NS>), grid, block, 0, stream, q, tiles_m, tiles_n, chunks_per_split);
   SDMI_HIP_OK(hipGetLastError());
   ps.end();
   if (nsplit > 1) return launch_splitk_reduce(q, nsplit, stream);
diff --git a/stable-diffusion_amd/csrc/igemm.hip b/stable-diffusion_amd/csrc/igemm.hip
--- a/stable-diffusion_amd/csrc/igemm.hip
+++ b/stable-diffusion_amd/csrc/igemm.hip
@@ -401,6 +401,7 @@
 static inline bool tile_tn_even(int t) { return (kTiles[t].bn / kTiles[t].wn / 32) % 2 == 0; }
 
 static int launch_tile(int tile, const IGemmParams& p, bool dma, int splitk, hipStream_t stream) {
+  if (p.tail_kt && !tile_is_halo(tile)) return fail("a GEMM with a 1x1 tail phase was routed to tile " + std::to_string(tile) + ": only the halo-staged conv tiles 14..17 run a tail");
   if (p.split16) return launch_split16_tile(tile, p, splitk, stream);
   if (igemm_has_half(p)) {
     switch (tile) {
@@ -421,9 +422,10 @@
 
 struct TuneKey {
   int M, N, K, ksize, stride, up, mode, splitk_req;
+  int kt = 0;
   bool operator<(const TuneKey& o) const {
-    return std::tie(M, N, K, ksize, stride, up, mode, splitk_req) <
-           std::tie(o.M, o.N, o.K, o.ksize, o.stride, o.up, o.mode, o.splitk_req);
+    return std::tie(M, N, K, ksize, stride, up, mode, splitk_req, kt) <
+           std::tie(o.M, o.N, o.K, o.ksize, o.stride, o.up, o.mode, o.splitk_req, o.kt);
   }
 };
 struct TuneChoice { int tile, splitk; double us; };
@@ -456,9 +458,10 @@
     while (fgets(line, sizeof line, f)) {
       if (line[0] == '#') continue;
       TuneKey k; TuneChoice c; c.us = 0;
-      if (sscanf(line, "%d %d %d %d %d %d %d %d %d %d %lf", &k.M, &k.N, &k.K, &k.ksize, &k.stride, &k.up, &k.mode,
-                 &k.splitk_req, &c.tile, &c.splitk, &c.us) >= 10 && c.tile >= 0 && c.tile < SDMI_NUM_TILES && c.splitk >= 1 &&
-          c.splitk <= 16)
+      k.kt = 0;
+      if (sscanf(line, "%d %d %d %d %d %d %d %d %d %d %lf %d", &k.M, &k.N, &k.K, &k.ksize, &k.stride, &k.up, &k.mode,
+                 &k.splitk_req, &c.tile, &c.splitk, &c.us, &k.kt) >= 10 && c.tile >= 0 && c.tile < SDMI_NUM_TILES && c.splitk >= 1 &&
+          c.splitk <= 16 && k.kt >= 0)
         table[k] = c;
     }
     fclose(f);
@@ -468,6 +471,11 @@
     loaded = true;
     if (env_int("SDMI_TUNE_DISABLE", 0)) return;
     load_file(default_path());
+  }
+  std::map<TuneKey, TuneChoice>::const_iterator find_entry(TuneKey k) const {
+    auto it = table.find(k);
+    if (it == table.end() && k.kt) { k.kt = 0; it = table.find(k); }
+    return it;
   }
   hipEvent_t ev() {
     if (!pool.empty()) { hipEvent_t e = pool.back(); pool.pop_back(); return e; }
@@ -485,6 +493,7 @@
   for (int t = 0; t < SDMI_NUM_TILES; ++t) {
     const TileCfg& c = kTiles[t];
     if (tile_is_halo(t) && !halo_supported(p, c.bm)) continue;
+    if (p.tail_kt && !tile_is_halo(t)) continue;
     if (p.split16 && !split16_tile_supported(t)) continue;
     if (!p.split16 && ((c.ns == 2 && t != 11 && !tile_is_halo(t)) || t == 12 || t == 13)) continue;
     if (p.mode == EPI_GEGLU && !tile_tn_even(t)) continue;
@@ -563,8 +572,10 @@
   fprintf(f, "# libsdmi igemm tuning table (gfx950), measured in situ by tools/tune.py -- M N K ksize stride up mode splitk_req tile splitk us\n");
   for (auto& kv : g_tuner.table) {
     const TuneKey& k = kv.first;
-    fprintf(f, "%d %d %d %d %d %d %d %d %d %d %.2f\n", k.M, k.N, k.K, k.ksize, k.stride, k.up, k.mode, k.splitk_req, kv.second.tile,
+    fprintf(f, "%d %d %d %d %d %d %d %d %d %d %.2f", k.M, k.N, k.K, k.ksize, k.stride, k.up, k.mode, k.splitk_req, kv.second.tile,
             kv.second.splitk, kv.second.us);
+    if (k.kt) fprintf(f, " %d", k.kt);
+    fprintf(f, "\n");
   }
   fclose(f);
   return 0;
@@ -578,12 +589,38 @@
       if (c.second.empty()) continue;
       std::vector<float> v = c.second;
       std::sort(v.begin(), v.end());
-      snprintf(buf, sizeof buf, "%d %d %d %d %d %d %d %d | %d %d %.2f %.2f %d\n", k.M, k.N, k.K, k.ksize, k.stride, k.up, k.mode,
-               k.splitk_req, c.first.tile, c.first.splitk, (double)v[v.size() / 2], (double)v[0], (int)v.size());
+      snprintf(buf, sizeof buf, "%d %d %d %d %d %d %d %d%s | %d %d %.2f %.2f %d\n", k.M, k.N, k.K, k.ksize, k.stride, k.up, k.mode,
+               k.splitk_req, k.kt ? (" t" + std::to_string(k.kt)).c_str() : "", c.first.tile, c.first.splitk, (double)v[v.size() / 2], (double)v[0], (int)v.size());
       *out += buf;
     }
   }
   return 0;
+}
+
+int tune_lookup(int M, int N, int K, int ksize, int stride, int up, int mode, int splitk_req, int kt, int* tile, int* splitk) {
+  std::lock_guard<std::mutex> lk(g_tuner.mu);
+  g_tuner.ensure_loaded();
+  auto it = g_tuner.find_entry(TuneKey{M, N, K, ksize, stride, up, mode, splitk_req, kt});
+  if (it == g_tuner.table.end()) return 1;
+  *tile = it->second.tile; *splitk = it->second.splitk;
+  return 0;
+}
+
+bool igemm_plans_halo(const IGemmParams& p) {
+  static const int env_tile = env_int("SDMI_IGEMM_TILE", -1);
+  if (p.ksize != 3 || p.split16 || igemm_has_half(p) || p.mode != EPI_PLAIN || p.splitk != 0 || env_tile >= 0 || env_int("SDMI_SPLITK", -1) >= 0) return false;
+  std::lock_guard<std::mutex> lk(g_tuner.mu);
+  g_tuner.ensure_loaded();
+  if (g_tuner.collecting) {
+    for (int t = 14; t <= 17; ++t) if (halo_supported(p, kTiles[t].bm)) return true;
+    return false;
+  }
+  auto it = g_tuner.find_entry(TuneKey{p.M, p.N, igemm_nkt(p) * BK, p.ksize, p.stride, p.up, p.mode, 0, p.tail_kt});
+  if (it == g_tuner.table.end()) return false;
+  const int tt = it->second.tile, sk = it->second.splitk, nkt = igemm_nkt(p);
+  const bool can_split = p.splitk_ws && p.N % 4 == 0 && p.ldo % 4 == 0 && (p.residual == nullptr || p.ldr % 4 == 0);
+  return tile_is_halo(tt) && halo_supported(p, kTiles[tt].bm) &&
+         (sk == 1 || (can_split && splitk_ws_need(p, kTiles[tt].bm, kTiles[tt].bn, sk) <= p.splitk_ws_floats && nkt / sk >= 4 && (nkt / 9) % sk == 0));
 }
 
 int launch_igemm(const IGemmParams& p, const IGemmTune& tune, hipStream_t stream) {
@@ -639,7 +676,7 @@
   if (env_split >= 0 && splitk == 0) splitk = env_split;
 
   hipEvent_t ev0 = nullptr, ev1 = nullptr;
-  TuneKey tkey{p.M, p.N, nkt * BK, p.split16 ? 11 : p.ksize, p.stride, p.up, p.mode, splitk};
+  TuneKey tkey{p.M, p.N, nkt * BK, p.split16 ? 11 : p.ksize, p.stride, p.up, p.mode, splitk, p.tail_kt};
   int tcand = -1;
   if (tile < 0) {
     std::lock_guard<std::mutex> lk(g_tuner.mu);
@@ -654,7 +691,7 @@
       tile = cands[tcand].tile; splitk = cands[tcand].splitk;
       ev0 = g_tuner.ev(); ev1 = g_tuner.ev();
     } else {
-      auto it = g_tuner.table.find(tkey);
+      auto it = g_tuner.find_entry(tkey);
       if (it != g_tuner.table.end()) {
         const int tt = it->second.tile, sk = it->second.splitk;
         const bool halo = tile_is_halo(tt);
diff --git a/stable-diffusion_amd/csrc/unet.cpp b/stable-diffusion_amd/csrc/unet.cpp
--- a/stable-diffusion_amd/csrc/unet.cpp
+++ b/stable-diffusion_amd/csrc/unet.cpp
@@ -306,6 +306,16 @@
       return 0;
     })) return -1;
     SDMI_HIP_OK(hipDeviceSynchronize());
+    if (for_each_layer([&](Layer& L) -> int {
+      if (L.kind != L_RES || L.updown || L.cin == L.cout || !L.f32[5] || !L.f32[6]) return 0;
+      std::vector<float> b2((size_t)L.cout), bs((size_t)L.cout);
+      SDMI_HIP_OK(hipMemcpy(b2.data(), L.f32[5], b2.size() * sizeof(float), hipMemcpyDeviceToHost));
+      SDMI_HIP_OK(hipMemcpy(bs.data(), L.f32[6], bs.size() * sizeof(float), hipMemcpyDeviceToHost));
+      for (size_t i = 0; i < b2.size(); ++i) b2[i] += bs[i];
+      if (store_.alloc((void**)&L.bias_fold, b2.size() * sizeof(float))) return -1;
+      SDMI_HIP_OK(hipMemcpy(L.bias_fold, b2.data(), b2.size() * sizeof(float), hipMemcpyHostToDevice));
+      return 0;
+    })) return -1;
   }
   ++weights_gen_;
   finalized_ = true;
@@ -403,6 +413,8 @@
   bool st_tail_on = false;
   bool st_mid_ctx_on = false;
   bool ctx1_on = false;
+  bool skip_fold_on = false; int skip_fold_max_w = 64;
+  std::vector<int>* skip_fold_plan = nullptr;
   bool gn_conv_on = false;
   float* emb_all = nullptr;
   int emb_ld = 0;
@@ -462,11 +474,25 @@
       gemm(p);
     }
     const float* residual = x0.p;
+    IGemmParams tailp = IGemmParams();
     if (Cin != Cout) {
-      IGemmParams p = dense1x1(raw, raw_lo, M, Cin, L.w16[2], Cout, H * W, p1);
-      p.bias = L.f32[6]; p.out_f32 = out.p; p.ldo = Cout;
-      gemm(p);
-      residual = out.p;
+      bool fold = skip_fold_on && !u->full() && !p3 && !ss && !gc2 && !gn_conv_on && W <= skip_fold_max_w && Cin % 64 == 0 && (dry || L.bias_fold != nullptr);
+      if (fold) {
+        IGemmParams c2 = conv3(raw, Cout, H, W, H, W, 1, 0, L.w16[1], Cout);
+        c2.tail_a0 = raw; c2.tail_a1 = p1 ? raw_lo : nullptr; c2.tail_a2 = p1 ? raw : nullptr;
+        c2.tail_c = Cin; c2.tail_ld = Cin; c2.tail_w = L.w16[2]; c2.tail_kt = p1 ? 3 * Cin : Cin;
+        c2.out_f32 = out.p; c2.ldo = Cout;
+        c2.splitk_ws = splitk_ws; c2.splitk_ws_floats = splitk_ws_floats;
+        fold = igemm_plans_halo(c2);
+        if (fold) tailp = c2;
+      }
+      if (skip_fold_plan && dry) skip_fold_plan->push_back(fold ? 1 : 0);
+      if (!fold) {
+        IGemmParams p = dense1x1(raw, raw_lo, M, Cin, L.w16[2], Cout, H * W, p1);
+        p.bias = L.f32[6]; p.out_f32 = out.p; p.ldo = Cout;
+        gemm(p);
+        residual = out.p;
+      }
     }
     if (gc2) {
       IGemmParams p = conv3(nullptr, Cout, H, W, H, W, 1, 0, L.w16[1], Cout);
@@ -485,6 +511,11 @@
       IGemmParams p = conv3(a2, Cout, H, W, H, W, 1, 0, L.w16[1], Cout);
       if (p3) split3(p, a2, a2_lo, Cout);
       p.bias = L.f32[5]; p.residual = residual; p.ldr = Cout; p.out_f32 = out.p; p.ldo = Cout;
+      if (tailp.tail_kt) {
+        p.tail_a0 = tailp.tail_a0; p.tail_a1 = tailp.tail_a1; p.tail_a2 = tailp.tail_a2; p.tail_c = tailp.tail_c; p.tail_ld = tailp.tail_ld;
+        p.tail_w = tailp.tail_w; p.tail_kt = tailp.tail_kt;
+        p.bias = L.bias_fold; p.residual = nullptr; p.ldr = 0;
+      }
       attach_gn_targets(p, out);
       attach_f16_copy(p, out);
       gemm(p);
@@ -1039,6 +1070,12 @@
     f.ctx1_on = !(e_c1 && atoi(e_c1) == 0);
     const char* e_gc = getenv("SDMI_GN_CONV");
     f.gn_conv_on = e_gc ? atoi(e_gc) != 0 : false;
+    const char* e_sf = getenv("SDMI_SKIP_FOLD");
+    f.skip_fold_on = e_sf ? atoi(e_sf) != 0 : skip_fold_;
+    const char* e_sfw = getenv("SDMI_SKIP_FOLD_MAX_W");
+    f.skip_fold_max_w = e_sfw ? atoi(e_sfw) : skip_fold_max_w_;
+    skip_fold_plan_.clear();
+    f.skip_fold_plan = &skip_fold_plan_;
     if (full()) {
       f.ln_fold_on = f.ff_tail_on = f.st_head_on = f.st_mid_on = f.st_tail_on = f.st_mid_ctx_on = f.gn_conv_on = false;
     }
diff --git a/stable-diffusion_amd/csrc/unet.h b/stable-diffusion_amd/csrc/unet.h
--- a/stable-diffusion_amd/csrc/unet.h
+++ b/stable-diffusion_amd/csrc/unet.h
@@ -197,6 +197,7 @@
   f16* w16[3] = {nullptr, nullptr, nullptr};
   float* w32[1] = {nullptr};
   float* f32[7] = {nullptr, nullptr, nullptr, nullptr, nullptr, nullptr, nullptr};
+  float* bias_fold = nullptr;
   std::vector<TBlock> tb;
 };
 
@@ -249,6 +250,10 @@
   bool ln_fold_ = true; int ln_fold_min_rows_ = 512;
   bool ff_tail_ = true;
   bool st_head_ = true;
+  bool skip_fold_ = true; int skip_fold_max_w_ = 64;
+ public:
+  std::vector<int> skip_fold_plan_;
+ private:
 
   struct TapeKey {
     int B = 0, H = 0, W = 0, Lctx = 0, mode = 0;
```
